# pyani-plus/pyani-plus

Hardware: AMD Instinct MI355X
Metric: pairwise genome comparisons/sec (N x N ANI matrix) (higher is better)
Workload: dtype u64

## Files before the change

pyani_plus_amd/csrc/capi.hip:

```cpp
#include <algorithm>
#include <cstdarg>
#include <cstring>

#include "pa_internal.h"

static thread_local char g_err[1024] = "";

void pa_set_error(const char *fmt, ...) {
  va_list ap;
  va_start(ap, fmt);
  vsnprintf(g_err, sizeof(g_err), fmt, ap);
  va_end(ap);
}

static hipEvent_t take_event(pa_ctx *c) {
  if (!c->event_pool.empty()) {
    hipEvent_t e = c->event_pool.back();
    c->event_pool.pop_back();
    return e;
  }
  hipEvent_t e = nullptr;
  if (hipEventCreate(&e) != hipSuccess) return nullptr;
  return e;
}

ProfScope::ProfScope(pa_ctx *ctx, int ph) : c(ctx), phase(ph) {
  if (!c->prof_on) return;
  e0 = take_event(c);
  e1 = take_event(c);
  if (e0) (void)hipEventRecord(e0, c->stream);
}

ProfScope::~ProfScope() {
  if (!c->prof_on || !e0 || !e1) return;
  (void)hipEventRecord(e1, c->stream);
  c->prof[phase].pending.emplace_back(e0, e1);
}

extern "C" {

int pa_abi_version(void) { return PA_ABI_VERSION; }
const char *pa_last_error(void) { return g_err; }

int pa_device_count(void) {
  int n = 0;
  if (hipGetDeviceCount(&n) != hipSuccess) return 0;
  return n;
}

int pa_ctx_create(int device, pa_ctx **out) {
  PA_REQUIRE(out != nullptr, "pa_ctx_create: out is null");
  *out = nullptr;
  int n = 0;
  hipError_t e = hipGetDeviceCount(&n);
  if (e != hipSuccess || n <= 0) {
    pa_set_error("no HIP device available (%s); libpyani_hip has no CPU fallback",
                 e != hipSuccess ? hipGetErrorString(e) : "device count is 0");
    return PA_E_NODEVICE;
  }
  PA_REQUIRE(device >= 0 && device < n, "pa_ctx_create: device %d out of range [0,%d)", device, n);
  PA_HIP(hipSetDevice(device));
  pa_ctx *c = new (std::nothrow) pa_ctx();
  if (!c) { pa_set_error("out of host memory"); return PA_E_NOMEM; }
  c->device = device;
  if (hipGetDeviceProperties(&c->prop, device) != hipSuccess) { delete c; pa_set_error("hipGetDeviceProperties failed"); return PA_E_HIP; }
  if (strncmp(c->prop.gcnArchName, "gfx950", 6) != 0) {
    pa_set_error("device %d is %s; this library is built for gfx950 (MI355X) only", device, c->prop.gcnArchName);
    delete c;
    return PA_E_NODEVICE;
  }
  if (hipStreamCreateWithFlags(&c->stream, hipStreamNonBlocking) != hipSuccess) { delete c; pa_set_error("hipStreamCreate failed"); return PA_E_HIP; }
  c->own_stream = true;
  if (hipHostMalloc(reinterpret_cast<void **>(&c->h_pinned), 64, hipHostMallocDefault) != hipSuccess) {
    (void)hipStreamDestroy(c->stream); delete c; pa_set_error("hipHostMalloc failed"); return PA_E_NOMEM;
  }
  if (c->counters.reserve(64) != PA_OK) { (void)hipHostFree(c->h_pinned); (void)hipStreamDestroy(c->stream); delete c; return PA_E_NOMEM; }
  *out = c;
  return PA_OK;
}

void pa_ctx_destroy(pa_ctx *c) {
  if (!c) return;
  (void)hipSetDevice(c->device);
  (void)hipStreamSynchronize(c->stream);
  DevBuf *bufs[] = {&c->cand_keys[0], &c->cand_keys[1], &c->cand_vals[0], &c->cand_vals[1], &c->genome_blk,
                    &c->counters, &c->hist, &c->flags, &c->scan_tmp, &c->region_off, &c->region_cursor, &c->dirty, &c->dict_keys[0], &c->dict_keys[1],
                    &c->dict_vals[0], &c->dict_vals[1], &c->ids, &c->post_genome, &c->bitrows, &c->dict_scalars, &c->cls_i, &c->cls_j, &c->cls_score,
                    &c->cls_cov};
  for (DevBuf *b : bufs) b->release();
  pa_fragani_release(c);
  for (auto &ph : c->prof)
    for (auto &pr : ph.pending) { (void)hipEventDestroy(pr.first); (void)hipEventDestroy(pr.second); }
  for (hipEvent_t e : c->event_pool) (void)hipEventDestroy(e);
  if (c->h_pinned) (void)hipHostFree(c->h_pinned);
  if (c->copy_stream) { (void)hipStreamSynchronize(c->copy_stream); (void)hipStreamDestroy(c->copy_stream); c->copy_stream = nullptr; }
  if (c->own_stream && c->stream) (void)hipStreamDestroy(c->stream);
  delete c;
}

int pa_ctx_set_stream(pa_ctx *c, void *hip_stream) {
  PA_REQUIRE(c != nullptr, "null context");
  PA_HIP(hipStreamSynchronize(c->stream));
  if (c->own_stream && c->stream) (void)hipStreamDestroy(c->stream);
  c->stream = reinterpret_cast<hipStream_t>(hip_stream);
  c->own_stream = false;
  return PA_OK;
}

int pa_ctx_own_stream(pa_ctx *c) {
  PA_REQUIRE(c != nullptr, "null context");
  if (c->own_stream) return PA_OK;
  PA_HIP(hipStreamSynchronize(c->stream));
  PA_HIP(hipStreamCreateWithFlags(&c->stream, hipStreamNonBlocking));
  c->own_stream = true;
  return PA_OK;
}

int pa_ctx_sync(pa_ctx *c) {
  PA_REQUIRE(c != nullptr, "null context");
  PA_HIP(hipStreamSynchronize(c->stream));
  return PA_OK;
}

int pa_ctx_device_info(pa_ctx *c, char *name256, int *compute_units, uint64_t *global_mem) {
  PA_REQUIRE(c != nullptr, "null context");
  if (name256) { snprintf(name256, 256, "%s (%s)", c->prop.name, c->prop.gcnArchName); }
  if (compute_units) *compute_units = c->prop.multiProcessorCount;
  if (global_mem) *global_mem = (uint64_t)c->prop.totalGlobalMem;
  return PA_OK;
}

int pa_dev_alloc(pa_ctx *c, uint64_t bytes, void **d_out) {
  PA_REQUIRE(c && d_out, "pa_dev_alloc: null argument");
  PA_HIP(hipSetDevice(c->device));
  hipError_t e = hipMalloc(d_out, bytes ? bytes : 16);
  if (e != hipSuccess) { pa_set_error("hipMalloc(%llu) failed: %s", (unsigned long long)bytes, hipGetErrorString(e)); return PA_E_NOMEM; }
  return PA_OK;
}
int pa_dev_free(pa_ctx *c, void *d_ptr) {
  PA_REQUIRE(c != nullptr, "null context");
  if (d_ptr) { PA_HIP(hipStreamSynchronize(c->stream)); PA_HIP(hipFree(d_ptr)); }
  return PA_OK;
}
int pa_memcpy_h2d(pa_ctx *c, void *d_dst, const void *h_src, uint64_t bytes) {
  PA_REQUIRE(c != nullptr, "null context");
  if (bytes == 0) return PA_OK;
  PA_HIP(hipMemcpyAsync(d_dst, h_src, bytes, hipMemcpyHostToDevice, c->stream));
  PA_HIP(hipStreamSynchronize(c->stream));
  return PA_OK;
}
int pa_memcpy_d2h(pa_ctx *c, void *h_dst, const void *d_src, uint64_t bytes) {
  PA_REQUIRE(c != nullptr, "null context");
  if (bytes == 0) return PA_OK;
  PA_HIP(hipMemcpyAsync(h_dst, d_src, bytes, hipMemcpyDeviceToHost, c->stream));
  PA_HIP(hipStreamSynchronize(c->stream));
  return PA_OK;
}
int pa_memset_d(pa_ctx *c, void *d_dst, int value, uint64_t bytes) {
  PA_REQUIRE(c != nullptr, "null context");
  if (bytes == 0) return PA_OK;
  PA_HIP(hipMemsetAsync(d_dst, value, bytes, c->stream));
  return PA_OK;
}

int pa_sketch(pa_ctx *c, const uint32_t *d_packed, const uint32_t *d_mask, const uint64_t *d_dirty_in, uint64_t arena_bases,
              const uint64_t *h_genome_start, uint32_t n_genomes, uint32_t k, uint64_t max_hash, uint64_t *d_hashes,
              uint64_t cap_hashes, uint64_t *d_off, uint64_t *h_total) {
  PA_REQUIRE(c && d_off && h_total && h_genome_start, "pa_sketch: null argument");
  PA_REQUIRE((arena_bases % PA_ALIGN_BASES) == 0, "pa_sketch: arena_bases %llu is not a multiple of %u",
             (unsigned long long)arena_bases, PA_ALIGN_BASES);
  PA_REQUIRE(arena_bases == 0 || (d_packed && d_mask), "pa_sketch: null arena");
  PA_REQUIRE(k >= 1 && k <= PA_MAX_K, "pa_sketch: k=%u outside [1,%u]", k, PA_MAX_K);
  PA_REQUIRE(h_genome_start[n_genomes] == arena_bases, "pa_sketch: genome_start[n] must equal arena_bases");
  PA_HIP(hipSetDevice(c->device));
  *h_total = 0;
  const uint64_t n_blocks = arena_bases / PA_ALIGN_BASES;
  std::vector<uint32_t> blk(n_genomes + 1);
  for (uint32_t g = 0; g <= n_genomes; ++g) {
    const uint64_t s = h_genome_start[g];
    PA_REQUIRE((s % PA_ALIGN_BASES) == 0 && (g == 0 || s >= h_genome_start[g - 1]) && s <= arena_bases,
               "pa_sketch: genome_start[%u]=%llu must be an ascending multiple of %u inside the arena", g,
               (unsigned long long)s, PA_ALIGN_BASES);
    blk[g] = (uint32_t)(s / PA_ALIGN_BASES);
  }
  PA_REQUIRE(n_blocks < (1ULL << 32), "pa_sketch: arena too large");
  PA_TRY(c->genome_blk.reserve((uint64_t)(n_genomes + 1) * sizeof(uint32_t)));
  PA_HIP(hipMemcpyAsync(c->genome_blk.p, blk.data(), (uint64_t)(n_genomes + 1) * sizeof(uint32_t),
                        hipMemcpyHostToDevice, c->stream));
  const double frac = (max_hash == UINT64_MAX) ? 1.0 : ((double)max_hash + 1.0) / 18446744073709551616.0;
  static const bool force_global = [] {
    const char *v = PA_TOOL_ENV("PA_SKETCH_SORT");
    return v && v[0] == 'g';
  }();
  std::vector<uint64_t> region_off(n_genomes + 1, 0);
  uint64_t longest_region = 0;
  for (uint32_t g = 0; g < n_genomes; ++g) {
    const uint64_t room = (uint64_t)((double)(h_genome_start[g + 1] - h_genome_start[g]) * frac * 1.25) + 128;
    longest_region = std::max(longest_region, room);
    region_off[g + 1] = region_off[g] + room;
  }
  const bool use_regions = !force_global && n_genomes > 0 && longest_region <= kLdsSortMax;
  if (use_regions) {
    PA_TRY(c->region_off.reserve((uint64_t)(n_genomes + 1) * sizeof(uint64_t)));
    PA_TRY(c->region_cursor.reserve((uint64_t)n_genomes * sizeof(uint32_t)));
    PA_HIP(hipMemcpyAsync(c->region_off.p, region_off.data(), (uint64_t)(n_genomes + 1) * sizeof(uint64_t),
                          hipMemcpyHostToDevice, c->stream));
  }
  const uint64_t *d_dirty = nullptr;
  PA_TRY(pa_dirty_or_build(c, d_mask, n_blocks, d_dirty_in, &d_dirty));
  PA_HIP(hipStreamSynchronize(c->stream));

  if (use_regions) {
    uint32_t *d_overflow = c->counters.as<uint32_t>() + 12;
    PA_TRY(c->cand_keys[0].reserve(region_off[n_genomes] * sizeof(uint64_t)));
    PA_HIP(hipMemsetAsync(c->region_cursor.p, 0, (uint64_t)n_genomes * sizeof(uint32_t), c->stream));
    PA_HIP(hipMemsetAsync(d_overflow, 0, sizeof(uint32_t), c->stream));
    {
      ProfScope prof(c, PA_PROF_KMER_HASH);
      PA_TRY(pa_launch_kmer_hash(c, d_packed, d_mask, d_dirty, n_blocks, c->genome_blk.as<uint32_t>(), n_genomes, k, max_hash,
                                 c->cand_keys[0].as<uint64_t>(), nullptr, 0, nullptr, c->region_off.as<uint64_t>(),
                                 c->region_cursor.as<uint32_t>(), d_overflow));
    }
    bool overflow = false;
    {
      ProfScope prof(c, PA_PROF_SKETCH_SORT);
      const int st = pa_sketch_from_regions(c, c->cand_keys[0].as<uint64_t>(), c->region_off.as<uint64_t>(),
                                            c->region_cursor.as<uint32_t>(), d_overflow, n_genomes,
                                            (uint32_t)longest_region, max_hash, d_hashes, cap_hashes, d_off, h_total, &overflow);
      if (st != PA_OK) return st;
    }
    if (!overflow) return PA_OK;
    *h_total = 0;
  }
  uint64_t cap = (uint64_t)((double)arena_bases * frac * 1.25) + 65536;
  if (cap > arena_bases) cap = arena_bases;
  uint64_t *d_count = c->counters.as<uint64_t>();
  uint64_t n_cand = 0;
  for (int attempt = 0; attempt < 2; ++attempt) {
    for (int b = 0; b < 2; ++b) {
      PA_TRY(c->cand_keys[b].reserve(cap * sizeof(uint64_t)));
      PA_TRY(c->cand_vals[b].reserve(cap * sizeof(uint32_t)));
    }
    PA_HIP(hipMemsetAsync(d_count, 0, sizeof(uint64_t), c->stream));
    {
      ProfScope prof(c, PA_PROF_KMER_HASH);
      PA_TRY(pa_launch_kmer_hash(c, d_packed, d_mask, d_dirty, n_blocks, c->genome_blk.as<uint32_t>(), n_genomes, k, max_hash,
                                 c->cand_keys[0].as<uint64_t>(), c->cand_vals[0].as<uint32_t>(), cap, d_count));
    }
    PA_HIP(hipMemcpyAsync(c->h_pinned, d_count, sizeof(uint64_t), hipMemcpyDeviceToHost, c->stream));
    PA_HIP(hipStreamSynchronize(c->stream));
    n_cand = c->h_pinned[0];
    if (n_cand <= cap) break;
    PA_REQUIRE(attempt == 0, "pa_sketch: candidate count changed between runs (%llu > %llu)",
               (unsigned long long)n_cand, (unsigned long long)cap);
    cap = n_cand;
  }
  {
    ProfScope prof(c, PA_PROF_SKETCH_SORT);
    uint64_t *keys[2] = {c->cand_keys[0].as<uint64_t>(), c->cand_keys[1].as<uint64_t>()};
    uint32_t *vals[2] = {c->cand_vals[0].as<uint32_t>(), c->cand_vals[1].as<uint32_t>()};
    int which = 0;
    int hash_bits = max_hash ? 64 - __builtin_clzll(max_hash) : 0;
    hash_bits = (hash_bits + 7) & ~7;
    int genome_bits = n_genomes > 1 ? 32 - __builtin_clz(n_genomes - 1) : 0;
    genome_bits = (genome_bits + 7) & ~7;
    PA_TRY(pa_radix_sort_pairs(c, keys, vals, n_cand, 0, hash_bits, false, &which));
    PA_TRY(pa_radix_sort_pairs(c, keys, vals, n_cand, 0, genome_bits, true, &which));
    int st = pa_build_sketch_csr(c, keys[which], vals[which], n_cand, n_genomes, d_hashes, cap_hashes, d_off, h_total);
    if (st != PA_OK) return st;
  }
  return PA_OK;
}

int pa_pair_counts_ex(pa_ctx *c, const uint64_t *d_hashes, const uint64_t *d_off, const uint64_t *h_off, uint32_t n,
                      uint32_t q0, uint32_t q1, uint32_t s0, uint32_t s1, uint32_t *d_counts, int algo) {
  PA_REQUIRE(c && d_off, "pa_pair_counts: null argument");
  PA_REQUIRE(q0 <= q1 && q1 <= n && s0 <= s1 && s1 <= n, "pa_pair_counts: ranges [%u,%u) x [%u,%u) outside [0,%u)", q0,
             q1, s0, s1, n);
  PA_REQUIRE(algo == PA_PAIRS_AUTO || algo == PA_PAIRS_BITROW || algo == PA_PAIRS_MERGE || algo == PA_PAIRS_BITROW_HASH,
             "pa_pair_counts: unknown algo %d", algo);
  PA_HIP(hipSetDevice(c->device));
  if (q0 == q1 || s0 == s1) { c->dict_prepared = false; return PA_OK; }
  PA_REQUIRE(d_counts != nullptr, "pa_pair_counts: null counts buffer");
  uint64_t total = 0;
  if (h_off) {
    total = h_off[n];
  } else {
    PA_HIP(hipMemcpyAsync(c->h_pinned, d_off + n, sizeof(uint64_t), hipMemcpyDeviceToHost, c->stream));
    PA_HIP(hipStreamSynchronize(c->stream));
    total = c->h_pinned[0];
  }
  PA_REQUIRE(total == 0 || d_hashes, "pa_pair_counts: null hashes");
  if (algo != PA_PAIRS_AUTO && algo != PA_PAIRS_BITROW_HASH) c->dict_prepared = false;
  switch (algo) {
    case PA_PAIRS_AUTO:
    case PA_PAIRS_BITROW_HASH:
      return pa_pairs_bitrow_hash(c, d_hashes, d_off, h_off, n, total, q0, q1, s0, s1, d_counts);
    case PA_PAIRS_BITROW:
      return pa_pairs_bitrow(c, d_hashes, d_off, n, total, q0, q1, s0, s1, d_counts);
    case PA_PAIRS_MERGE:
      return pa_pairs_merge(c, d_hashes, d_off, n, q0, q1, s0, s1, d_counts);
    default:
      pa_set_error("pa_pair_counts: unknown algo %d", algo);
      return PA_E_INVALID;
  }
}

int pa_pair_counts(pa_ctx *c, const uint64_t *d_hashes, const uint64_t *d_off, uint32_t n, uint32_t q0, uint32_t q1,
                   uint32_t s0, uint32_t s1, uint32_t *d_counts, int algo) {
  return pa_pair_counts_ex(c, d_hashes, d_off, nullptr, n, q0, q1, s0, s1, d_counts, algo);
}

int pa_pair_dict_prepare(pa_ctx *c, const uint64_t *d_subject_hashes, uint64_t n_postings) {
  PA_REQUIRE(c && (n_postings == 0 || d_subject_hashes), "pa_pair_dict_prepare: null argument");
  PA_HIP(hipSetDevice(c->device));
  return pa_pair_dict_prepare_impl(c, d_subject_hashes, n_postings);
}

int pa_ani(pa_ctx *c, const uint32_t *d_counts, const uint64_t *d_off, uint32_t q0, uint32_t q1, uint32_t s0,
           uint32_t s1, uint32_t k, double *d_identity, double *d_cov_query) {
  PA_REQUIRE(c && d_counts && d_off && d_identity && d_cov_query, "pa_ani: null argument");
  PA_REQUIRE(k >= 1 && q0 <= q1 && s0 <= s1, "pa_ani: bad k or ranges");
  PA_HIP(hipSetDevice(c->device));
  return pa_launch_ani(c, d_counts, d_off, q0, q1, s0, s1, k, d_identity, d_cov_query);
}

int pa_prof_enable(pa_ctx *c, int on) {
  PA_REQUIRE(c != nullptr, "null context");
  c->prof_on = on != 0;
  return PA_OK;
}

static int prof_drain(pa_ctx *c) {
  PA_HIP(hipStreamSynchronize(c->stream));
  for (auto &ph : c->prof) {
    for (auto &pr : ph.pending) {
      float ms = 0.f;
      if (hipEventElapsedTime(&ms, pr.first, pr.second) == hipSuccess) {
        ph.total_ms += ms;
        ph.launches += 1;
      }
      c->event_pool.push_back(pr.first);
      c->event_pool.push_back(pr.second);
    }
    ph.pending.clear();
  }
  return PA_OK;
}

int pa_prof_reset(pa_ctx *c) {
  PA_REQUIRE(c != nullptr, "null context");
  PA_TRY(prof_drain(c));
  for (auto &ph : c->prof) { ph.total_ms = 0.0; ph.launches = 0; }
  return PA_OK;
}

int pa_prof_get(pa_ctx *c, int phase, double *total_ms, uint64_t *launches) {
  PA_REQUIRE(c != nullptr && phase >= 0 && phase < PA_PROF_NPHASES, "pa_prof_get: bad phase %d", phase);
  PA_TRY(prof_drain(c));
  if (total_ms) *total_ms = c->prof[phase].total_ms;
  if (launches) *launches = c->prof[phase].launches;
  return PA_OK;
}

}
```

pyani_plus_amd/csrc/kmer_hash.hip:

```cpp
#include <cstdlib>
#include <type_traits>

#include "pa_internal.h"
#include "murmur_dev.h"

namespace {

using namespace pa_dev;

constexpr int kThreads = 256;
constexpr uint32_t kStageCap = 1024;

constexpr int pow2_floor(int k) { int c = 1; while (2 * c <= k) c *= 2; return c; }

__device__ __forceinline__ uint32_t find_genome(const uint32_t *__restrict__ genome_blk, uint32_t n, uint32_t blk) {
  uint32_t lo = 0, hi = n;
  while (hi - lo > 1) {
    uint32_t mid = (lo + hi) >> 1;
    if (genome_blk[mid] <= blk) lo = mid; else hi = mid;
  }
  return lo;
}

__device__ __forceinline__ void region_append(uint64_t *__restrict__ regions, const uint64_t *__restrict__ region_off,
                                              uint32_t *__restrict__ cursor, uint32_t *__restrict__ overflow,
                                              uint32_t g, uint64_t h) {
  const uint64_t slot = atomicAdd(&cursor[g], 1u);
  if (slot < region_off[g + 1] - region_off[g]) regions[region_off[g] + slot] = h; else *overflow = 1u;
}

template <int K, bool LUT>
__global__ __launch_bounds__(kThreads) void kmer_hash_kernel(
    const uint4 *__restrict__ packed, const uint2 *__restrict__ mask, const uint64_t *__restrict__ dirty, uint32_t n_blocks64,
    const uint32_t *__restrict__ genome_blk, uint32_t n_genomes, uint64_t max_hash,
    uint64_t *__restrict__ cand_hash, uint32_t *__restrict__ cand_genome, uint64_t cap,
    unsigned long long *__restrict__ count, const uint64_t *__restrict__ region_off, uint32_t *__restrict__ cursor,
    uint32_t *__restrict__ overflow, uint32_t blk0) {
  static_assert(K >= 1 && K <= 32, "a k-mer is one 64-bit register pair");
  __shared__ uint64_t s_hash[kStageCap];
  __shared__ uint32_t s_blk[kStageCap];
  __shared__ uint32_t s_n;
  __shared__ unsigned long long s_base;
  constexpr int kWords = (K + 7) / 8;
  __shared__ uint64_t s_lo[LUT ? kWords : 1][256];
  __shared__ uint32_t s_hi[LUT ? kWords : 1][256];

  const uint32_t tid = threadIdx.x;
  const uint32_t max_hi = (uint32_t)(max_hash >> 32);
  const bool take_all = max_hi == 0xffffffffu;
  const uint32_t screen_hi = max_hi + 1u;
  if (tid == 0) s_n = 0;
  if constexpr (LUT) {
#pragma unroll
    for (int j = 0; j < kWords; ++j) {
      const uint64_t cj = (j & 1) ? kC2 : kC1;
      s_lo[j][tid] = (uint64_t)ascii_group(tid, K - 8 * j) * cj;
      s_hi[j][tid] = (uint32_t)((uint64_t)ascii_group(tid, K - 8 * j - 4) * cj);
    }
  }
  __syncthreads();

  const uint32_t t = blk0 + blockIdx.x * kThreads + tid;
  if (t < n_blocks64) {
    const uint4 cur = packed[t];
    uint2 pw = make_uint2(0u, 0u);
    if (t > 0) pw = reinterpret_cast<const uint2 *>(packed)[2 * (uint64_t)t - 1];
    uint32_t d1 = 0u, d2 = 0u;
    const uint32_t wave_blk = __builtin_amdgcn_readfirstlane(t & ~63u);
    const uint64_t dirty_word = dirty[wave_blk >> 6];
    if ((dirty_word >> (t & 63u)) & 1ull) {
      const uint2 m = mask[t];
      uint32_t d0 = t > 0 ? mask[t - 1].y : 0xffffffffu;
      d1 = m.x;
      d2 = m.y;
      int c = 1;
#pragma unroll
      for (; 2 * c <= K; c *= 2) {
        d2 |= alignbit(d2, d1, 32 - c);
        d1 |= alignbit(d1, d0, 32 - c);
        d0 |= d0 << c;
      }
      constexpr int cc = pow2_floor(K);
      constexpr int r = K - cc;
      if constexpr (r > 0) {
        d2 |= alignbit(d2, d1, 32 - r);
        d1 |= alignbit(d1, d0, 32 - r);
      }
    }
    const uint32_t bad[2] = {d1, d2};
    if ((d1 & d2) != 0xffffffffu) {
      constexpr uint64_t kMask = (K == 32) ? ~0ULL : ((1ULL << (2 * K)) - 1);
      constexpr uint32_t kMaskHi = (uint32_t)(kMask >> 32);
      uint32_t fw[8] = {pw.x, pw.y, cur.x, cur.y, cur.z, cur.w, 0u, 0u};
      uint32_t rw[6];
#pragma unroll
      for (int j = 0; j < 6; ++j) {
        const uint32_t x = __builtin_bitreverse32(fw[5 - j]);
        rw[j] = ~(((x >> 1) & 0x55555555u) | ((x & 0x55555555u) << 1));
      }
      auto columns = [&](auto base_tag, int i_begin, int i_end) {
        constexpr int kBase = decltype(base_tag)::value;
#pragma unroll 1
        for (int i = i_begin; i < i_end; ++i) {
          constexpr int kOff = 33 - K;
          const uint32_t fo = 2u * (uint32_t)((i + kOff) & 15), ro = 30u - 2u * (uint32_t)i;
          uint32_t A[5], B[5];
#pragma unroll
          for (int j = 0; j < 5; ++j) {
            A[j] = alignbit(fw[kBase + j + 1], fw[kBase + j], fo);
            B[j] = alignbit(rw[j + 1], rw[j], ro);
          }
#pragma unroll
          for (int wi = 0; wi < 4; ++wi) {
            const uint32_t f_lo = A[wi], f_hi = A[wi + 1], r_lo = B[3 - wi], r_hi = B[4 - wi];
          const uint64_t f_lsb = u64_of(f_lo, f_hi) & kMask, r_lsb = u64_of(r_lo, r_hi) & kMask;
          const uint64_t fwd = __builtin_amdgcn_uicmpl(f_lsb, r_lsb, 37 );
          uint32_t clo, chi;
          asm("s_nop 1\n\tv_cndmask_b32_e64 %0, %1, %2, %3" : "=v"(clo) : "v"((uint32_t)r_lsb), "v"((uint32_t)f_lsb), "s"(fwd));
          asm("v_cndmask_b32_e64 %0, %1, %2, %3" : "=v"(chi) : "v"((uint32_t)(r_lsb >> 32)), "v"((uint32_t)(f_lsb >> 32)), "s"(fwd), "v"(clo));
          uint64_t P[4] = {0, 0, 0, 0};
#pragma unroll
          for (int j = 0; j < kWords; ++j) {
            const uint32_t src = j < 2 ? clo : chi;
            const uint32_t glo = (src >> (16 * (j & 1))) & 0xffu, ghi = (src >> (16 * (j & 1) + 8)) & 0xffu;
            if constexpr (LUT) {
              const uint64_t lo = s_lo[j][glo];
              const uint32_t hi = (uint32_t)(lo >> 32) + s_hi[j][ghi];
              P[j] = u64_of((uint32_t)lo, hi);
            } else {
              const uint64_t word = u64_of(ascii_group(glo, K - 8 * j), ascii_group(ghi, K - 8 * j - 4));
              P[j] = word * ((j & 1) ? kC2 : kC1);
            }
          }
          (void)kMaskHi;
          uint64_t U, V;
          murmur3_pre_last_mul<K>(P, U, V);
          if (take_all || last_mul_high_sum_plus1(U, V) <= screen_hi) {
            const uint64_t X = U * kF2, Y = V * kF2;
            const uint64_t h = (X ^ (X >> 33)) + (Y ^ (Y >> 33));
            if (h > max_hash || ((bad[wi >> 1] >> (16 * (wi & 1) + i)) & 1u)) continue;
            const uint32_t slot = atomicAdd(&s_n, 1u);
            if (slot < kStageCap) {
              s_hash[slot] = h;
              s_blk[slot] = t;
            } else if (region_off) {
              region_append(cand_hash, region_off, cursor, overflow, find_genome(genome_blk, n_genomes, t), h);
            } else {
              const unsigned long long g = atomicAdd(count, 1ULL);
              if (g < cap) {
                cand_hash[g] = h;
                cand_genome[g] = find_genome(genome_blk, n_genomes, t);
              }
            }
          }
          }
        }
      };
      constexpr int kOff0 = 33 - K, kSplit = (kOff0 & 15) ? 16 - (kOff0 & 15) : 16;
      columns(std::integral_constant<int, (kOff0 >> 4)>{}, 0, kSplit);
      if constexpr (kSplit < 16) columns(std::integral_constant<int, (kOff0 >> 4) + 1>{}, kSplit, 16);
    }
  }
  __syncthreads();
  const uint32_t n = min(s_n, kStageCap);
  if (n == 0) return;
  if (region_off) {
    const uint32_t b0 = blk0 + blockIdx.x * kThreads;
    const uint32_t b1 = min(b0 + (uint32_t)kThreads, n_blocks64) - 1u;
    const uint32_t g0 = find_genome(genome_blk, n_genomes, b0);
    if (genome_blk[g0 + 1] > b1) {
      if (tid == 0) s_base = atomicAdd(&cursor[g0], n);
      __syncthreads();
      const uint64_t room = region_off[g0 + 1] - region_off[g0];
      uint64_t *__restrict__ dst = cand_hash + region_off[g0];
      for (uint32_t i = tid; i < n; i += kThreads) {
        const uint64_t slot = s_base + i;
        if (slot < room) dst[slot] = s_hash[i]; else *overflow = 1u;
      }
    } else {
      for (uint32_t i = tid; i < n; i += kThreads)
        region_append(cand_hash, region_off, cursor, overflow, find_genome(genome_blk, n_genomes, s_blk[i]), s_hash[i]);
    }
    return;
  }
  if (tid == 0) s_base = atomicAdd(count, (unsigned long long)n);
  __syncthreads();
  const unsigned long long base = s_base;
  for (uint32_t i = tid; i < n; i += kThreads) {
    const unsigned long long g = base + i;
    if (g < cap) {
      cand_hash[g] = s_hash[i];
      cand_genome[g] = find_genome(genome_blk, n_genomes, s_blk[i]);
    }
  }
}

template <int K, bool LUT>
int launch_variant(pa_ctx *c, const uint32_t *d_packed, const uint32_t *d_mask, const uint64_t *d_dirty, uint64_t n_blocks64,
           const uint32_t *d_genome_blk, uint32_t n_genomes, uint64_t max_hash, uint64_t *d_cand_hash,
           uint32_t *d_cand_genome, uint64_t cap, uint64_t *d_count, const uint64_t *d_region_off, uint32_t *d_cursor,
           uint32_t *d_overflow, uint64_t blk0, hipStream_t stream) {
  const uint32_t grid = ceil_div_u64(n_blocks64 - blk0, kThreads);
  hipLaunchKernelGGL((kmer_hash_kernel<K, LUT>), dim3(grid), dim3(kThreads), 0, stream ? stream : c->stream,
                     reinterpret_cast<const uint4 *>(d_packed), reinterpret_cast<const uint2 *>(d_mask), d_dirty,
                     (uint32_t)n_blocks64, d_genome_blk, n_genomes, max_hash, d_cand_hash, d_cand_genome, cap,
                     reinterpret_cast<unsigned long long *>(d_count), d_region_off, d_cursor, d_overflow, (uint32_t)blk0);
  PA_HIP(hipGetLastError());
  return PA_OK;
}

template <int K>
int launch(pa_ctx *c, const uint32_t *d_packed, const uint32_t *d_mask, const uint64_t *d_dirty, uint64_t n_blocks64,
           const uint32_t *d_genome_blk, uint32_t n_genomes, uint64_t max_hash, uint64_t *d_cand_hash,
           uint32_t *d_cand_genome, uint64_t cap, uint64_t *d_count, const uint64_t *d_region_off, uint32_t *d_cursor,
           uint32_t *d_overflow, uint64_t blk0, hipStream_t stream) {
  static const bool arithmetic = [] {
    const char *v = PA_TOOL_ENV("PA_KMER_VARIANT");
    return v && v[0] == '0';
  }();
  if constexpr (K == 31)
    if (arithmetic)
      return launch_variant<K, false>(c, d_packed, d_mask, d_dirty, n_blocks64, d_genome_blk, n_genomes, max_hash, d_cand_hash,
                                    d_cand_genome, cap, d_count, d_region_off, d_cursor, d_overflow, blk0, stream);
  return launch_variant<K, true>(c, d_packed, d_mask, d_dirty, n_blocks64, d_genome_blk, n_genomes, max_hash, d_cand_hash,
                                 d_cand_genome, cap, d_count, d_region_off, d_cursor, d_overflow, blk0, stream);
}

template <int K>
__global__ __launch_bounds__(kThreads) void kmer_hash_wide_kernel(
    const uint4 *__restrict__ packed, const uint2 *__restrict__ mask, const uint64_t *__restrict__ dirty, uint32_t n_blocks64,
    const uint32_t *__restrict__ genome_blk, uint32_t n_genomes, uint64_t max_hash,
    uint64_t *__restrict__ cand_hash, uint32_t *__restrict__ cand_genome, uint64_t cap,
    unsigned long long *__restrict__ count, const uint64_t *__restrict__ region_off, uint32_t *__restrict__ cursor,
    uint32_t *__restrict__ overflow, uint32_t blk0) {
  static_assert(K >= 33 && K <= 64, "k-mers of 65 to 128 bits");
  __shared__ uint64_t s_hash[kStageCap];
  __shared__ uint32_t s_blk[kStageCap];
  __shared__ uint32_t s_n;
  __shared__ unsigned long long s_base;
  constexpr int kWords = (K + 7) / 8;
  __shared__ uint64_t s_lo[kWords][256];
  __shared__ uint32_t s_hi[kWords][256];
  const uint32_t tid = threadIdx.x;
  const uint32_t max_hi = (uint32_t)(max_hash >> 32);
  const bool take_all = max_hi == 0xffffffffu;
  const uint32_t screen_hi = max_hi + 1u;
  if (tid == 0) s_n = 0;
#pragma unroll
  for (int j = 0; j < kWords; ++j) {
    const uint64_t cj = (j & 1) ? kC2 : kC1;
    s_lo[j][tid] = (uint64_t)ascii_group(tid, K - 8 * j) * cj;
    s_hi[j][tid] = (uint32_t)((uint64_t)ascii_group(tid, K - 8 * j - 4) * cj);
  }
  __syncthreads();

  const uint32_t t = blk0 + blockIdx.x * kThreads + tid;
  if (t < n_blocks64) {
    const uint4 cur = packed[t];
    const uint4 prev = t > 0 ? packed[t - 1] : make_uint4(0u, 0u, 0u, 0u);
    uint32_t d2 = 0u, d3 = 0u;
    const uint32_t wave_blk = __builtin_amdgcn_readfirstlane(t & ~63u);
    const uint64_t dirty_word = dirty[wave_blk >> 6];
    const uint64_t before = wave_blk ? dirty[(wave_blk >> 6) - 1] >> 63 : 1ull;
    const uint64_t dirty_or_prev = dirty_word | (dirty_word << 1) | before;
    if ((dirty_or_prev >> (t & 63u)) & 1ull) {
      const uint2 m = mask[t];
      uint32_t d0 = 0xffffffffu, d1 = 0xffffffffu;
      if (t > 0) { const uint2 mp = mask[t - 1]; d0 = mp.x; d1 = mp.y; }
      d2 = m.x;
      d3 = m.y;
#pragma unroll
      for (int c = 1; c <= 16; c *= 2) {
        d3 |= alignbit(d3, d2, 32 - c);
        d2 |= alignbit(d2, d1, 32 - c);
        d1 |= alignbit(d1, d0, 32 - c);
        d0 |= d0 << c;
      }
      if constexpr (K == 64) {
        d3 |= d2; d2 |= d1; d1 |= d0;
      } else {
        constexpr int r = K - 32;
        d3 |= alignbit(d3, d2, 32 - r);
        d2 |= alignbit(d2, d1, 32 - r);
        d1 |= alignbit(d1, d0, 32 - r);
      }
    }
    const uint32_t bad[2] = {d2, d3};
    if ((d2 & d3) != 0xffffffffu) {
      constexpr uint32_t kMask2 = (2 * K - 64 >= 32) ? 0xffffffffu : ((1u << (2 * K - 64)) - 1u);
      constexpr uint32_t kMask3 = (2 * K - 96 >= 32) ? 0xffffffffu : (2 * K - 96 <= 0 ? 0u : ((1u << ((2 * K - 96) & 31)) - 1u));
      const uint32_t fw[10] = {prev.x, prev.y, prev.z, prev.w, cur.x, cur.y, cur.z, cur.w, 0u, 0u};
      uint32_t rw[10];
#pragma unroll
      for (int j = 0; j < 10; ++j) {
        const uint32_t x = __builtin_bitreverse32(fw[9 - j]);
        rw[j] = ~(((x >> 1) & 0x55555555u) | ((x & 0x55555555u) << 1));
      }
      auto columns = [&](auto base_tag, int i_begin, int i_end) {
        constexpr int kBase = decltype(base_tag)::value;
#pragma unroll 1
        for (int i = i_begin; i < i_end; ++i) {
          constexpr int kOff = 65 - K;
          const uint32_t fo = 2u * (uint32_t)((i + kOff) & 15), ro = 30u - 2u * (uint32_t)i;
          uint32_t A[7], B[7];
#pragma unroll
          for (int j = 0; j < 7; ++j) {
            A[j] = alignbit(fw[kBase + j + 1], fw[kBase + j], fo);
            B[j] = alignbit(rw[j + 3], rw[j + 2], ro);
          }
#pragma unroll
          for (int wi = 0; wi < 4; ++wi) {
            const uint32_t f0 = A[wi], f1 = A[wi + 1], f2 = A[wi + 2] & kMask2, f3 = A[wi + 3] & kMask3;
            const uint32_t r0 = B[3 - wi], r1 = B[4 - wi], r2 = B[5 - wi] & kMask2, r3 = B[6 - wi] & kMask3;
            const uint64_t lt_hi = __builtin_amdgcn_uicmpl(u64_of(f2, f3), u64_of(r2, r3), 36 );
            const uint64_t eq_hi = __builtin_amdgcn_uicmpl(u64_of(f2, f3), u64_of(r2, r3), 32 );
            const uint64_t le_lo = __builtin_amdgcn_uicmpl(u64_of(f0, f1), u64_of(r0, r1), 37 );
            const uint64_t fwd = lt_hi | (eq_hi & le_lo);
            uint32_t c0, c1, c2, c3;
            asm("s_nop 1\n\tv_cndmask_b32_e64 %0, %1, %2, %3" : "=v"(c0) : "v"(r0), "v"(f0), "s"(fwd));
            asm("v_cndmask_b32_e64 %0, %1, %2, %3" : "=v"(c1) : "v"(r1), "v"(f1), "s"(fwd), "v"(c0));
            asm("v_cndmask_b32_e64 %0, %1, %2, %3" : "=v"(c2) : "v"(r2), "v"(f2), "s"(fwd), "v"(c1));
            asm("v_cndmask_b32_e64 %0, %1, %2, %3" : "=v"(c3) : "v"(r3), "v"(f3), "s"(fwd), "v"(c2));
            const uint32_t cw[4] = {c0, c1, c2, c3};
            uint64_t P[8] = {0, 0, 0, 0, 0, 0, 0, 0};
#pragma unroll
            for (int j = 0; j < kWords; ++j) {
              const uint32_t src = cw[j >> 1];
              const uint32_t glo = (src >> (16 * (j & 1))) & 0xffu, ghi = (src >> (16 * (j & 1) + 8)) & 0xffu;
              const uint64_t lo = s_lo[j][glo];
              P[j] = u64_of((uint32_t)lo, (uint32_t)(lo >> 32) + s_hi[j][ghi]);
            }
            uint64_t U, V;
            murmur3_pre_last_mul<K>(P, U, V);
            if (take_all || last_mul_high_sum_plus1(U, V) <= screen_hi) {
              const uint64_t X = U * kF2, Y = V * kF2;
              const uint64_t h = (X ^ (X >> 33)) + (Y ^ (Y >> 33));
              if (h > max_hash || ((bad[wi >> 1] >> (16 * (wi & 1) + i)) & 1u)) continue;
              const uint32_t slot = atomicAdd(&s_n, 1u);
              if (slot < kStageCap) {
                s_hash[slot] = h;
                s_blk[slot] = t;
              } else if (region_off) {
                region_append(cand_hash, region_off, cursor, overflow, find_genome(genome_blk, n_genomes, t), h);
              } else {
                const unsigned long long g = atomicAdd(count, 1ULL);
                if (g < cap) {
                  cand_hash[g] = h;
                  cand_genome[g] = find_genome(genome_blk, n_genomes, t);
                }
              }
            }
          }
        }
      };
      constexpr int kOff0 = 65 - K, kSplit = (kOff0 & 15) ? 16 - (kOff0 & 15) : 16;
      columns(std::integral_constant<int, (kOff0 >> 4)>{}, 0, kSplit);
      if constexpr (kSplit < 16) columns(std::integral_constant<int, (kOff0 >> 4) + 1>{}, kSplit, 16);
    }
  }
  __syncthreads();
  const uint32_t n = min(s_n, kStageCap);
  if (n == 0) return;
  if (region_off) {
    const uint32_t b0 = blk0 + blockIdx.x * kThreads;
    const uint32_t b1 = min(b0 + (uint32_t)kThreads, n_blocks64) - 1u;
    const uint32_t g0 = find_genome(genome_blk, n_genomes, b0);
    if (genome_blk[g0 + 1] > b1) {
      if (tid == 0) s_base = atomicAdd(&cursor[g0], n);
      __syncthreads();
      const uint64_t room = region_off[g0 + 1] - region_off[g0];
      uint64_t *__restrict__ dst = cand_hash + region_off[g0];
      for (uint32_t i = tid; i < n; i += kThreads) {
        const uint64_t slot = s_base + i;
        if (slot < room) dst[slot] = s_hash[i]; else *overflow = 1u;
      }
    } else {
      for (uint32_t i = tid; i < n; i += kThreads)
        region_append(cand_hash, region_off, cursor, overflow, find_genome(genome_blk, n_genomes, s_blk[i]), s_hash[i]);
    }
    return;
  }
  if (tid == 0) s_base = atomicAdd(count, (unsigned long long)n);
  __syncthreads();
  const unsigned long long base = s_base;
  for (uint32_t i = tid; i < n; i += kThreads) {
    const unsigned long long g = base + i;
    if (g < cap) {
      cand_hash[g] = s_hash[i];
      cand_genome[g] = find_genome(genome_blk, n_genomes, s_blk[i]);
    }
  }
}

__device__ __forceinline__ uint32_t rev_groups32(uint32_t x) {
  x = __builtin_bitreverse32(x);
  return ((x >> 1) & 0x55555555u) | ((x & 0x55555555u) << 1);
}

__device__ __forceinline__ void murmur3_pre_last_mul_rt(const uint64_t (&P)[8], uint32_t k, uint64_t &U, uint64_t &V) {
  uint64_t h1 = 42, h2 = 42;
  const uint32_t nblocks = k >> 4, tail = k & 15u;
#pragma unroll
  for (uint32_t i = 0; i < 4; ++i) {
    if (i >= nblocks) break;
    h1 ^= rotl64(P[2 * i], 31) * kC2;
    h1 = rotl64(h1, 27) + h2;
    h1 = times5_plus(h1, 0x52dce729ULL);
    h2 ^= rotl64(P[2 * i + 1], 33) * kC1;
    h2 = rotl64(h2, 31) + h1;
    h2 = times5_plus(h2, 0x38495ab5ULL);
  }
  uint64_t t1 = 0, t2 = 0;
#pragma unroll
  for (uint32_t i = 0; i < 4; ++i)
    if (i == nblocks) { t1 = P[2 * i]; t2 = P[2 * i + 1]; }
  if (tail > 8) h2 ^= rotl64(t2, 33) * kC1;
  if (tail > 0) h1 ^= rotl64(t1, 31) * kC2;
  h1 ^= (uint64_t)k;
  h2 ^= (uint64_t)k;
  h1 += h2;
  h2 += h1;
  h1 ^= h1 >> 33; h1 *= kF1; h1 ^= h1 >> 33;
  h2 ^= h2 >> 33; h2 *= kF1; h2 ^= h2 >> 33;
  U = h1;
  V = h2;
}

constexpr int kLongIter = 32;
__global__ __launch_bounds__(kThreads) void kmer_hash_long_kernel(
    const uint32_t *__restrict__ packed, const uint32_t *__restrict__ mask, uint64_t pos0, uint64_t pos1, uint32_t k,
    const uint32_t *__restrict__ genome_blk, uint32_t n_genomes, uint64_t max_hash, uint64_t *__restrict__ cand_hash,
    uint32_t *__restrict__ cand_genome, uint64_t cap, unsigned long long *__restrict__ count,
    const uint64_t *__restrict__ region_off, uint32_t *__restrict__ cursor, uint32_t *__restrict__ overflow) {
  __shared__ uint64_t s_lo[8][256];
  __shared__ uint32_t s_hi[8][256];
  const uint32_t tid = threadIdx.x;
  const uint32_t n_words = (k + 7u) >> 3;
  for (uint32_t j = 0; j < n_words; ++j) {
    const uint64_t cj = (j & 1u) ? kC2 : kC1;
    s_lo[j][tid] = (uint64_t)ascii_group(tid, (int)k - 8 * (int)j) * cj;
    s_hi[j][tid] = (uint32_t)((uint64_t)ascii_group(tid, (int)k - 8 * (int)j - 4) * cj);
  }
  __syncthreads();
  const uint64_t wg_first = pos0 + ((uint64_t)blockIdx.y * gridDim.x + blockIdx.x) * (uint64_t)(kThreads * kLongIter);
#pragma unroll 1
  for (int it = 0; it < kLongIter; ++it) {
  const uint64_t e = wg_first + (uint64_t)it * kThreads + tid;
  if (e >= pos1 || e + 1 < k) continue;
  const uint64_t a = e + 1 - k;
  {
    const uint64_t m0 = a >> 5, m_last = e >> 5;
    const uint32_t sm = (uint32_t)(a & 31u);
    const uint32_t w0 = mask[m0], w1 = m0 + 1 <= m_last ? mask[m0 + 1] : 0u, w2 = m0 + 2 <= m_last ? mask[m0 + 2] : 0u;
    const uint32_t b0 = alignbit(w1, w0, sm), b1 = alignbit(w2, w1, sm);
    const uint32_t top = k == 64 ? 0xffffffffu : ((1u << (k - 32u)) - 1u);
    if (b0 | (b1 & top)) continue;
  }
  uint32_t F[4], R[4];
  {
    const uint64_t p0 = a >> 4, p_last = e >> 4;
    const uint32_t sp = 2u * (uint32_t)(a & 15u);
    uint32_t w[5];
#pragma unroll
    for (int i = 0; i < 5; ++i) w[i] = p0 + i <= p_last ? packed[p0 + i] : 0u;
#pragma unroll
    for (int i = 0; i < 4; ++i) F[i] = alignbit(w[i + 1], w[i], sp);
    const uint32_t used = 2u * k - 64u;
    if (used < 32u) { F[2] &= (1u << used) - 1u; F[3] = 0u; }
    else if (used < 64u) F[3] &= (1u << (used - 32u)) - 1u;
    const uint32_t C[6] = {~rev_groups32(F[3]), ~rev_groups32(F[2]), ~rev_groups32(F[1]), ~rev_groups32(F[0]), 0u, 0u};
    const uint32_t s = 128u - 2u * k, ws = s >> 5, bs = s & 31u;
#pragma unroll
    for (int i = 0; i < 4; ++i) R[i] = ws ? alignbit(C[i + 2], C[i + 1], bs) : alignbit(C[i + 1], C[i], bs);
    if (used < 32u) { R[2] &= (1u << used) - 1u; R[3] = 0u; }
    else if (used < 64u) R[3] &= (1u << (used - 32u)) - 1u;
  }
  const uint64_t f_hi = u64_of(F[2], F[3]), f_lo = u64_of(F[0], F[1]), r_hi = u64_of(R[2], R[3]), r_lo = u64_of(R[0], R[1]);
  const bool fwd = f_hi < r_hi || (f_hi == r_hi && f_lo <= r_lo);
  uint32_t c[4];
#pragma unroll
  for (int i = 0; i < 4; ++i) c[i] = fwd ? F[i] : R[i];
  uint64_t P[8] = {0, 0, 0, 0, 0, 0, 0, 0};
#pragma unroll
  for (uint32_t j = 0; j < 8; ++j) {
    if (j >= n_words) break;
    const uint32_t src = c[j >> 1], glo = (src >> (16u * (j & 1u))) & 0xffu, ghi = (src >> (16u * (j & 1u) + 8u)) & 0xffu;
    const uint64_t lo = s_lo[j][glo];
    P[j] = u64_of((uint32_t)lo, (uint32_t)(lo >> 32) + s_hi[j][ghi]);
  }
  uint64_t U, V;
  murmur3_pre_last_mul_rt(P, k, U, V);
  const uint32_t max_hi = (uint32_t)(max_hash >> 32);
  if (max_hi != 0xffffffffu && last_mul_high_sum_plus1(U, V) > max_hi + 1u) continue;
  const uint64_t X = U * kF2, Y = V * kF2;
  const uint64_t h = (X ^ (X >> 33)) + (Y ^ (Y >> 33));
  if (h > max_hash) continue;
  const uint32_t blk = (uint32_t)(e >> 6);
  const uint32_t g = find_genome(genome_blk, n_genomes, blk);
  if (region_off) {
    region_append(cand_hash, region_off, cursor, overflow, g, h);
  } else {
    const unsigned long long slot = atomicAdd(count, 1ULL);
    if (slot < cap) {
      cand_hash[slot] = h;
      cand_genome[slot] = g;
    }
  }
  }
}

}

int pa_launch_kmer_hash(pa_ctx *c, const uint32_t *d_packed, const uint32_t *d_mask, const uint64_t *d_dirty, uint64_t n_blocks64,
                        const uint32_t *d_genome_blk, uint32_t n_genomes, uint32_t k, uint64_t max_hash,
                        uint64_t *d_cand_hash, uint32_t *d_cand_genome, uint64_t cap, uint64_t *d_count,
                        const uint64_t *d_region_off, uint32_t *d_cursor, uint32_t *d_overflow, uint64_t blk0,
                        hipStream_t stream) {
  PA_REQUIRE(n_blocks64 < (1ULL << 32), "arena too large: %llu blocks of 64 bases", (unsigned long long)n_blocks64);
  if (n_blocks64 <= blk0) return PA_OK;
  const char *long_form = PA_TOOL_ENV("PA_KMER_LONG");
  const bool long_plain = long_form && long_form[0] == 'p';
  if (k > 32 && k <= 64 && !long_plain) {
    PA_REQUIRE((blk0 & 63u) == 0, "k-mer hash launch must start at a multiple of 64 blocks, not %llu", (unsigned long long)blk0);
    const uint32_t grid = ceil_div_u64(n_blocks64 - blk0, kThreads);
#define PA_WIDE_CASE(KK)                                                                                                   \
  case KK:                                                                                                                 \
    hipLaunchKernelGGL((kmer_hash_wide_kernel<KK>), dim3(grid), dim3(kThreads), 0, stream ? stream : c->stream,            \
                       reinterpret_cast<const uint4 *>(d_packed), reinterpret_cast<const uint2 *>(d_mask), d_dirty,        \
                       (uint32_t)n_blocks64, d_genome_blk, n_genomes, max_hash, d_cand_hash, d_cand_genome, cap,           \
                       reinterpret_cast<unsigned long long *>(d_count), d_region_off, d_cursor, d_overflow, (uint32_t)blk0); \
    break;
    switch (k) {
      PA_WIDE_CASE(33) PA_WIDE_CASE(34) PA_WIDE_CASE(35) PA_WIDE_CASE(36) PA_WIDE_CASE(37) PA_WIDE_CASE(38) PA_WIDE_CASE(39)
      PA_WIDE_CASE(40) PA_WIDE_CASE(41) PA_WIDE_CASE(42) PA_WIDE_CASE(43) PA_WIDE_CASE(44) PA_WIDE_CASE(45) PA_WIDE_CASE(46)
      PA_WIDE_CASE(47) PA_WIDE_CASE(48) PA_WIDE_CASE(49) PA_WIDE_CASE(50) PA_WIDE_CASE(51) PA_WIDE_CASE(52) PA_WIDE_CASE(53)
      PA_WIDE_CASE(54) PA_WIDE_CASE(55) PA_WIDE_CASE(56) PA_WIDE_CASE(57) PA_WIDE_CASE(58) PA_WIDE_CASE(59) PA_WIDE_CASE(60)
      PA_WIDE_CASE(61) PA_WIDE_CASE(62) PA_WIDE_CASE(63) PA_WIDE_CASE(64)
      default: break;
    }
#undef PA_WIDE_CASE
    PA_HIP(hipGetLastError());
    return PA_OK;
  }
  if (k > 32 && k <= 64) {
    const uint64_t pos0 = blk0 * 64, pos1 = n_blocks64 * 64;
    const uint64_t per_wg = (uint64_t)kThreads * kLongIter;
    const uint64_t n_wg = (pos1 - pos0 + per_wg - 1) / per_wg;
    const uint32_t gx = (uint32_t)std::min<uint64_t>(n_wg, 1u << 20), gy = (uint32_t)((n_wg + gx - 1) / gx);
    PA_REQUIRE(gy <= 65535u, "arena too large for one launch of the long k-mer kernel: %llu positions", (unsigned long long)(pos1 - pos0));
    hipLaunchKernelGGL(kmer_hash_long_kernel, dim3(gx, gy), dim3(kThreads), 0,
                       stream ? stream : c->stream, d_packed, d_mask, pos0, pos1, k, d_genome_blk, n_genomes, max_hash,
                       d_cand_hash, d_cand_genome, cap, reinterpret_cast<unsigned long long *>(d_count), d_region_off,
                       d_cursor, d_overflow);
    PA_HIP(hipGetLastError());
    return PA_OK;
  }
#define PA_K_CASE(KK) \
  case KK: return launch<KK>(c, d_packed, d_mask, d_dirty, n_blocks64, d_genome_blk, n_genomes, max_hash, d_cand_hash, d_cand_genome, cap, d_count, d_region_off, d_cursor, d_overflow, blk0, stream);
  PA_REQUIRE((blk0 & 63u) == 0, "k-mer hash launch must start at a multiple of 64 blocks, not %llu", (unsigned long long)blk0);
  switch (k) {
    PA_K_CASE(1) PA_K_CASE(2) PA_K_CASE(3) PA_K_CASE(4) PA_K_CASE(5) PA_K_CASE(6) PA_K_CASE(7) PA_K_CASE(8)
    PA_K_CASE(9) PA_K_CASE(10) PA_K_CASE(11) PA_K_CASE(12) PA_K_CASE(13) PA_K_CASE(14) PA_K_CASE(15) PA_K_CASE(16)
    PA_K_CASE(17) PA_K_CASE(18) PA_K_CASE(19) PA_K_CASE(20) PA_K_CASE(21) PA_K_CASE(22) PA_K_CASE(23) PA_K_CASE(24)
    PA_K_CASE(25) PA_K_CASE(26) PA_K_CASE(27) PA_K_CASE(28) PA_K_CASE(29) PA_K_CASE(30) PA_K_CASE(31) PA_K_CASE(32)
    default:
      pa_set_error("k=%u outside [1,64]", k);
      return PA_E_INVALID;
  }
#undef PA_K_CASE
}
```

pyani_plus_amd/csrc/murmur_dev.h:

```cpp
#pragma once

#include <hip/hip_runtime.h>

#include <cstdint>

namespace pa_dev {

__device__ __forceinline__ uint32_t alignbit(uint32_t hi, uint32_t lo, uint32_t sh) {
  return __builtin_amdgcn_alignbit(hi, lo, sh);
}

__device__ __forceinline__ uint32_t ascii4(uint32_t b8) {
  uint32_t u = (b8 | (b8 << 12)) & 0x000F000Fu;
  uint32_t v = (u | (u << 6)) & 0x03030303u;
  return __builtin_amdgcn_perm(0u, 0x54474341u, v);
}

__device__ __forceinline__ uint64_t u64_of(uint32_t lo, uint32_t hi) { return ((uint64_t)hi << 32) | lo; }

__device__ __forceinline__ uint64_t rotl64(uint64_t x, int r) {
  const uint32_t lo = (uint32_t)x, hi = (uint32_t)(x >> 32);
  if (r == 32) return u64_of(hi, lo);
  if (r < 32) return u64_of(alignbit(lo, hi, 32 - r), alignbit(hi, lo, 32 - r));
  return u64_of(alignbit(hi, lo, 64 - r), alignbit(lo, hi, 64 - r));
}

__device__ __forceinline__ uint64_t fmix64(uint64_t k) {
  k ^= k >> 33;
  k *= 0xff51afd7ed558ccdULL;
  k ^= k >> 33;
  k *= 0xc4ceb9fe1a85ec53ULL;
  k ^= k >> 33;
  return k;
}

constexpr uint64_t kC1 = 0x87c37b91114253d5ULL, kC2 = 0x4cf5ad432745937fULL;

__device__ __forceinline__ uint64_t times5_plus(uint64_t h, uint64_t c) {
  uint64_t t;
  asm("v_lshl_add_u64 %0, %1, 2, %1" : "=v"(t) : "v"(h));
  return t + c;
}

constexpr uint64_t kF1 = 0xff51afd7ed558ccdULL, kF2 = 0xc4ceb9fe1a85ec53ULL;

template <int K, int N>
__device__ __forceinline__ void murmur3_pre_last_mul(const uint64_t (&P)[N], uint64_t &U, uint64_t &V) {
  static_assert(N >= (K + 7) / 8, "one first product per 8-byte word of the k-mer");
  uint64_t h1 = 42, h2 = 42;
  constexpr int nblocks = K / 16;
  constexpr int tail = K % 16;
#pragma unroll
  for (int i = 0; i < nblocks; ++i) {
    const uint64_t k1 = rotl64(P[2 * i], 31) * kC2;
    h1 ^= k1;
    if (i == 0) {
      h1 = times5_plus(rotl64(h1, 27), 5ULL * 42ULL + 0x52dce729ULL);
    } else {
      h1 = rotl64(h1, 27) + h2;
      h1 = times5_plus(h1, 0x52dce729ULL);
    }
    const uint64_t k2 = rotl64(P[2 * i + 1], 33) * kC1;
    h2 ^= k2;
    h2 = rotl64(h2, 31) + h1;
    h2 = times5_plus(h2, 0x38495ab5ULL);
  }
  if constexpr (tail > 8) h2 ^= rotl64(P[2 * nblocks + 1], 33) * kC1;
  if constexpr (tail > 0) h1 ^= rotl64(P[2 * nblocks], 31) * kC2;
  h1 ^= (uint64_t)K; h2 ^= (uint64_t)K;
  h1 += h2; h2 += h1;
  h1 ^= h1 >> 33; h1 *= kF1; h1 ^= h1 >> 33;
  h2 ^= h2 >> 33; h2 *= kF1; h2 ^= h2 >> 33;
  U = h1;
  V = h2;
}

__device__ __forceinline__ uint32_t last_mul_high_sum_plus1(uint64_t U, uint64_t V) {
  constexpr uint32_t c0 = (uint32_t)kF2, c1 = (uint32_t)(kF2 >> 32);
  const uint32_t u0 = (uint32_t)U, u1 = (uint32_t)(U >> 32), v0 = (uint32_t)V, v1 = (uint32_t)(V >> 32);
  return (__umulhi(u0, c0) + __umulhi(v0, c0) + 1u) + ((u0 + v0) * c1 + (u1 + v1) * c0);
}

template <int K, int N>
__device__ __forceinline__ uint64_t murmur3_from_products(const uint64_t (&P)[N]) {
  uint64_t U, V;
  murmur3_pre_last_mul<K, N>(P, U, V);
  const uint64_t X = U * kF2, Y = V * kF2;
  return (X ^ (X >> 33)) + (Y ^ (Y >> 33));
}

__device__ __forceinline__ uint32_t ascii_group(uint32_t b8, int nv) {
  const uint32_t a = ascii4(b8);
  return nv >= 4 ? a : (nv <= 0 ? 0u : (a & ((1u << (8 * nv)) - 1u)));
}

}
```

pyani_plus_amd/csrc/pa_internal.h:

```cpp
#pragma once

#include <hip/hip_runtime.h>

#include <cstdarg>
#include <cstdint>
#include <cstdio>
#include <string>
#include <vector>

#include "../../include/pyani_hip.h"

void pa_set_error(const char *fmt, ...);

#define PA_HIP(call)                                                                          \
  do {                                                                                        \
    hipError_t _e = (call);                                                                   \
    if (_e != hipSuccess) {                                                                   \
      pa_set_error("%s failed: %s (%s:%d)", #call, hipGetErrorString(_e), __FILE__, __LINE__); \
      return PA_E_HIP;                                                                        \
    }                                                                                         \
  } while (0)

#define PA_TRY(call)          \
  do {                        \
    int _s = (call);          \
    if (_s != PA_OK) return _s; \
  } while (0)

#define PA_REQUIRE(cond, ...)   \
  do {                          \
    if (!(cond)) {              \
      pa_set_error(__VA_ARGS__); \
      return PA_E_INVALID;      \
    }                           \
  } while (0)

#ifdef PA_TOOLS
#include <cstdlib>
#define PA_TOOL_ENV(name) getenv(name)
#else
#define PA_TOOL_ENV(name) static_cast<const char *>(nullptr)
#endif

struct DevBudget {
  uint64_t held = 0, peak = 0, cap = 0;
  char what[192] = {0};
};
struct DevBuf {
  void *p = nullptr;
  uint64_t bytes = 0;
  DevBudget *budget = nullptr;
  int reserve(uint64_t want) {
    if (want <= bytes) return PA_OK;
    uint64_t sz = want + want / 4 + 256;
    if (budget && budget->cap && budget->held - bytes + sz > budget->cap) {
      pa_set_error("%s: the workspace would grow to %llu bytes (%llu held; this buffer from %llu to %llu), above the cap of %llu bytes",
                   budget->what[0] ? budget->what : "device workspace", (unsigned long long)(budget->held - bytes + sz),
                   (unsigned long long)budget->held, (unsigned long long)bytes, (unsigned long long)sz, (unsigned long long)budget->cap);
      return PA_E_NOMEM;
    }
    if (p) (void)hipFree(p);
    if (budget) budget->held -= bytes;
    p = nullptr;
    bytes = 0;
    hipError_t e = hipMalloc(&p, sz);
    if (e != hipSuccess) {
      if (budget)
        pa_set_error("%s: hipMalloc(%llu) failed with %llu bytes of workspace held: %s", budget->what[0] ? budget->what : "device workspace",
                     (unsigned long long)sz, (unsigned long long)budget->held, hipGetErrorString(e));
      else
        pa_set_error("hipMalloc(%llu) failed: %s", (unsigned long long)sz, hipGetErrorString(e));
      p = nullptr;
      return PA_E_NOMEM;
    }
    bytes = sz;
    if (budget) {
      budget->held += sz;
      if (budget->held > budget->peak) budget->peak = budget->held;
    }
    return PA_OK;
  }
  void release() {
    if (p) (void)hipFree(p);
    if (budget) budget->held -= bytes;
    p = nullptr;
    bytes = 0;
  }
  template <typename T>
  T *as() const { return reinterpret_cast<T *>(p); }
};

struct ProfPhase {
  double total_ms = 0.0;
  uint64_t launches = 0;
  std::vector<std::pair<hipEvent_t, hipEvent_t>> pending;
};

struct pa_ctx {
  int device = 0;
  hipStream_t stream = nullptr;
  bool own_stream = false;
  hipDeviceProp_t prop;
  DevBuf cand_keys[2], cand_vals[2];
  DevBuf genome_blk;
  DevBuf counters;
  DevBuf hist;
  DevBuf flags, scan_tmp;
  DevBuf region_off, region_cursor;
  DevBuf dirty;
  DevBuf dict_keys[2], dict_vals[2];
  DevBuf ids, post_genome, bitrows;
  bool dict_prepared = false;
  uint64_t dict_prepared_postings = 0;
  uint32_t dict_prepared_cap = 0;
  DevBuf dict_scalars;
  hipStream_t copy_stream = nullptr;
  DevBuf cls_i, cls_j, cls_score, cls_cov;
  void *frag_work = nullptr;
  uint64_t *h_pinned = nullptr;
  bool prof_on = false;
  ProfPhase prof[PA_PROF_NPHASES];
  std::vector<hipEvent_t> event_pool;
};

struct ProfScope {
  pa_ctx *c;
  int phase;
  hipEvent_t e0 = nullptr, e1 = nullptr;
  ProfScope(pa_ctx *ctx, int ph);
  ~ProfScope();
};

static inline uint32_t ceil_div_u64(uint64_t a, uint64_t b) { return (uint32_t)((a + b - 1) / b); }

int pa_radix_sort_pairs(pa_ctx *c, uint64_t *keys[2], uint32_t *vals[2], uint64_t n, int bit_lo,
                        int bit_hi, bool by_val, int *which);
int pa_exclusive_scan_u32(pa_ctx *c, const uint32_t *d_in, uint32_t *d_out, uint64_t n,
                          uint64_t *d_total_u64 );

void pa_fragani_release(pa_ctx *c);

int pa_launch_kmer_hash(pa_ctx *c, const uint32_t *d_packed, const uint32_t *d_mask, const uint64_t *d_dirty, uint64_t n_blocks64,
                        const uint32_t *d_genome_blk, uint32_t n_genomes, uint32_t k, uint64_t max_hash,
                        uint64_t *d_cand_hash, uint32_t *d_cand_genome, uint64_t cap, uint64_t *d_count,
                        const uint64_t *d_region_off = nullptr, uint32_t *d_cursor = nullptr,
                        uint32_t *d_overflow = nullptr, uint64_t blk0 = 0, hipStream_t stream = nullptr);

int pa_build_dirty(pa_ctx *c, const uint32_t *d_mask, uint64_t n_blocks64, uint64_t *d_dirty, hipStream_t stream = nullptr);
int pa_dirty_or_build(pa_ctx *c, const uint32_t *d_mask, uint64_t n_blocks64, const uint64_t *d_dirty, const uint64_t **out);

constexpr uint32_t kLdsSortMax = 16384;
int pa_sketch_from_regions(pa_ctx *c, uint64_t *d_regions, const uint64_t *d_region_off, const uint32_t *d_cursor,
                           const uint32_t *d_overflow, uint32_t n_genomes, uint32_t longest_region, uint64_t max_hash,
                           uint64_t *d_hashes, uint64_t cap_hashes, uint64_t *d_off, uint64_t *h_total, bool *h_overflow);

int pa_build_sketch_csr(pa_ctx *c, const uint64_t *d_sorted_hash, const uint32_t *d_sorted_genome,
                        uint64_t n_cand, uint32_t n_genomes, uint64_t *d_hashes, uint64_t cap_hashes,
                        uint64_t *d_off, uint64_t *h_total);

int pa_pairs_bitrow(pa_ctx *c, const uint64_t *d_hashes, const uint64_t *d_off, uint32_t n, uint64_t total,
                    uint32_t q0, uint32_t q1, uint32_t s0, uint32_t s1, uint32_t *d_counts);
int pa_dense_ids_sorted(pa_ctx *c, const uint64_t *d_hashes, const uint64_t *d_off, uint32_t n, uint64_t P,
                        uint64_t *n_distinct);
int pa_pairs_bitrow_hash(pa_ctx *c, const uint64_t *d_hashes, const uint64_t *d_off, const uint64_t *h_off ,
                         uint32_t n, uint64_t total, uint32_t q0, uint32_t q1, uint32_t s0, uint32_t s1,
                         uint32_t *d_counts);
int pa_pair_dict_prepare_impl(pa_ctx *c, const uint64_t *d_subject_hashes, uint64_t n_postings);
int pa_pairs_merge(pa_ctx *c, const uint64_t *d_hashes, const uint64_t *d_off, uint32_t n, uint32_t q0,
                   uint32_t q1, uint32_t s0, uint32_t s1, uint32_t *d_counts);

int pa_launch_ani(pa_ctx *c, const uint32_t *d_counts, const uint64_t *d_off, uint32_t q0, uint32_t q1,
                  uint32_t s0, uint32_t s1, uint32_t k, double *d_identity, double *d_cov_query);
```

pyani_plus_amd/csrc/pairs_bitrow.hip:

```cpp
#include <algorithm>
#include <cstdlib>
#include <vector>

#include "pa_internal.h"

namespace {

constexpr int kThreads = 256;
constexpr int kPlanes = 10;
constexpr uint32_t kMaxTileSubjects = 2048;
constexpr uint32_t kNone = 0xffffffffu;
constexpr uint64_t kEmptyKey = ~0ULL;

__global__ __launch_bounds__(kThreads) void iota_kernel(uint32_t *__restrict__ vals, uint64_t n) {
  const uint64_t i = (uint64_t)blockIdx.x * kThreads + threadIdx.x;
  if (i < n) vals[i] = (uint32_t)i;
}

__global__ __launch_bounds__(kThreads) void last_or_kernel(const uint64_t *__restrict__ hashes,
                                                           const uint64_t *__restrict__ off, uint32_t n,
                                                           unsigned long long *__restrict__ or_out) {
  const uint32_t g = blockIdx.x * kThreads + threadIdx.x;
  uint64_t k = 0;
  if (g < n && off[g + 1] > off[g]) k = hashes[off[g + 1] - 1];
#pragma unroll
  for (int o = 32; o > 0; o >>= 1) k |= __shfl_xor(k, o, 64);
  if ((threadIdx.x & 63u) == 0 && k) atomicOr(or_out, (unsigned long long)k);
}

__global__ __launch_bounds__(kThreads) void key_heads_kernel(const uint64_t *__restrict__ keys, uint64_t n,
                                                             uint32_t *__restrict__ flags) {
  const uint64_t i = (uint64_t)blockIdx.x * kThreads + threadIdx.x;
  if (i < n) flags[i] = (i == 0 || keys[i] != keys[i - 1]) ? 1u : 0u;
}

__device__ __forceinline__ uint32_t owner_of(const uint64_t *__restrict__ off, uint32_t n, uint64_t j) {
  uint32_t lo = 0, hi = n;
  while (hi - lo > 1) {
    const uint32_t mid = (lo + hi) >> 1;
    if (off[mid] <= j) lo = mid; else hi = mid;
  }
  return lo;
}

__global__ __launch_bounds__(kThreads) void assign_ids_kernel(
    const uint32_t *__restrict__ sorted_post, const uint32_t *__restrict__ flags, const uint32_t *__restrict__ pos,
    uint64_t n, const uint64_t *__restrict__ off, uint32_t n_genomes, uint32_t *__restrict__ ids_csr,
    uint32_t *__restrict__ id_sorted, uint32_t *__restrict__ genome_sorted) {
  const uint64_t i = (uint64_t)blockIdx.x * kThreads + threadIdx.x;
  if (i >= n) return;
  const uint32_t id = pos[i] + flags[i] - 1u;
  const uint32_t j = sorted_post[i];
  ids_csr[j] = id;
  id_sorted[i] = id;
  genome_sorted[i] = owner_of(off, n_genomes, j);
}

__global__ __launch_bounds__(kThreads) void build_rows_kernel(const uint32_t *__restrict__ id_sorted,
                                                              const uint32_t *__restrict__ genome_sorted, uint64_t n,
                                                              uint32_t t0, uint32_t t1, uint32_t w32,
                                                              uint32_t *__restrict__ rows) {
  const uint64_t i = (uint64_t)blockIdx.x * kThreads + threadIdx.x;
  if (i >= n) return;
  const uint32_t g = genome_sorted[i];
  if (g < t0 || g >= t1) return;
  const uint32_t col = g - t0;
  atomicOr(&rows[(uint64_t)id_sorted[i] * w32 + (col >> 5)], 1u << (col & 31u));
}

struct U4 { uint32_t v[4]; };

template <int TPR>
__global__ __launch_bounds__(kThreads) void row_sum_kernel(const uint32_t *__restrict__ ids_csr,
                                                           const uint64_t *__restrict__ off, uint32_t q0,
                                                           const uint32_t *__restrict__ rows, uint32_t tile_cols,
                                                           uint32_t *__restrict__ counts, uint32_t ns,
                                                           uint32_t col0) {
  constexpr int kRowsPerIter = kThreads / TPR;
  constexpr int kW32 = TPR * 4;
  __shared__ uint32_t s_cnt[kW32 * 32];
  const uint32_t tid = threadIdx.x;
  for (uint32_t x = tid; x < kW32 * 32; x += kThreads) s_cnt[x] = 0;
  __syncthreads();

  const uint32_t q = q0 + blockIdx.x;
  const uint64_t beg = off[q], len = off[q + 1] - beg;
  const uint32_t *__restrict__ ids = ids_csr + beg;
  const uint32_t slot = tid / TPR, quad = tid % TPR;

  uint32_t plane[kPlanes][4];
#pragma unroll
  for (int p = 0; p < kPlanes; ++p)
#pragma unroll
    for (int c = 0; c < 4; ++c) plane[p][c] = 0;
  uint32_t pending = 0;

  auto flush = [&]() {
#pragma unroll
    for (int c = 0; c < 4; ++c) {
      uint32_t any = 0;
#pragma unroll
      for (int p = 0; p < kPlanes; ++p) any |= plane[p][c];
      while (any) {
        const uint32_t b = (uint32_t)__builtin_ctz(any);
        any &= any - 1u;
        uint32_t v = 0;
#pragma unroll
        for (int p = 0; p < kPlanes; ++p) v |= ((plane[p][c] >> b) & 1u) << p;
        atomicAdd(&s_cnt[(quad * 4 + c) * 32 + b], v);
      }
    }
#pragma unroll
    for (int p = 0; p < kPlanes; ++p)
#pragma unroll
      for (int c = 0; c < 4; ++c) plane[p][c] = 0;
    pending = 0;
  };

  constexpr int kBatch = 8;
  auto csa = [](uint32_t &carry, uint32_t &sum, uint32_t a, uint32_t b, uint32_t c) {
    const uint32_t u = a ^ b;
    carry = (a & b) | (u & c);
    sum = u ^ c;
  };
  const uint64_t j_begin = slot < (uint32_t)kRowsPerIter ? slot : len;
  uint32_t id_next[kBatch];
#pragma unroll
  for (int u = 0; u < kBatch; ++u) {
    const uint64_t j = j_begin + (uint64_t)u * kRowsPerIter;
    id_next[u] = j < len ? ids[j] : kNone;
  }
  for (uint64_t j0 = j_begin; j0 < len; j0 += (uint64_t)kRowsPerIter * kBatch) {
    uint4 r[kBatch];
#pragma unroll
    for (int u = 0; u < kBatch; ++u) {
      const uint32_t id = id_next[u];
      r[u] = id != kNone ? *reinterpret_cast<const uint4 *>(rows + (uint64_t)id * kW32 + quad * 4) : make_uint4(0u, 0u, 0u, 0u);
    }
#pragma unroll
    for (int u = 0; u < kBatch; ++u) {
      const uint64_t j = j0 + (uint64_t)(kBatch + u) * kRowsPerIter;
      id_next[u] = j < len ? ids[j] : kNone;
    }
#pragma unroll
    for (int c = 0; c < 4; ++c) {
      auto word = [&](int u) -> uint32_t { return c == 0 ? r[u].x : c == 1 ? r[u].y : c == 2 ? r[u].z : r[u].w; };
      uint32_t twos_a, twos_b, fours_a, fours_b, eights;
      csa(twos_a, plane[0][c], plane[0][c], word(0), word(1));
      csa(twos_b, plane[0][c], plane[0][c], word(2), word(3));
      csa(fours_a, plane[1][c], plane[1][c], twos_a, twos_b);
      csa(twos_a, plane[0][c], plane[0][c], word(4), word(5));
      csa(twos_b, plane[0][c], plane[0][c], word(6), word(7));
      csa(fours_b, plane[1][c], plane[1][c], twos_a, twos_b);
      csa(eights, plane[2][c], plane[2][c], fours_a, fours_b);
#pragma unroll
      for (int p = 3; p < kPlanes; ++p) {
        const uint32_t t = plane[p][c] & eights;
        plane[p][c] ^= eights;
        eights = t;
      }
    }
    pending += kBatch;
    if (pending + kBatch > (1u << kPlanes) - 1u) flush();
  }
  if (pending) flush();
  __syncthreads();
  uint32_t *__restrict__ out = counts + (uint64_t)blockIdx.x * ns + col0;
  for (uint32_t x = tid; x < tile_cols; x += kThreads) out[x] = s_cnt[x];
}

__global__ __launch_bounds__(kThreads) void zero_rows_kernel(uint4 *__restrict__ rows, const uint32_t *__restrict__ d_u,
                                                             uint32_t w32) {
  const uint64_t n16 = ((uint64_t)(*d_u ? *d_u : 1u) * w32) / 4u;
  const uint64_t i = (uint64_t)blockIdx.x * kThreads + threadIdx.x;
  if (i < n16) rows[i] = make_uint4(0u, 0u, 0u, 0u);
}

struct DictEntry {
  unsigned long long key;
  uint32_t id;
  uint32_t pad;
};
static_assert(sizeof(DictEntry) == 16, "one probe = one 16-byte entry");

__device__ __forceinline__ uint32_t slot_of(uint64_t h, uint32_t cap) {
  const uint32_t x = ((uint32_t)h * 0x9E3779B1u) ^ (uint32_t)(h >> 32);
  return (uint32_t)(((uint64_t)x * cap) >> 32);
}

constexpr int kInsertPerThread = 4;
__global__ __launch_bounds__(kThreads) void table_insert_kernel(const uint64_t *__restrict__ hashes, uint64_t p0,
                                                                uint64_t p1, DictEntry *__restrict__ table,
                                                                uint32_t cap, uint32_t *__restrict__ counter,
                                                                uint32_t *__restrict__ special) {
  __shared__ uint32_t s_won, s_base;
  if (threadIdx.x == 0) s_won = 0;
  __syncthreads();
  uint32_t won_slot[kInsertPerThread];
  int won = 0;
  bool won_special = false;
  const uint64_t base = p0 + (uint64_t)blockIdx.x * (kThreads * kInsertPerThread) + threadIdx.x;
#pragma unroll
  for (int i = 0; i < kInsertPerThread; ++i) {
    const uint64_t p = base + (uint64_t)i * kThreads;
    if (p >= p1) break;
    const uint64_t h = hashes[p];
    if (h == kEmptyKey) {
      won_special = atomicCAS(&special[0], kNone, kNone - 1u) == kNone;
      continue;
    }
    uint32_t slot = slot_of(h, cap);
    for (;;) {
      unsigned long long k = *reinterpret_cast<volatile const unsigned long long *>(&table[slot].key);
      if (k == kEmptyKey) k = atomicCAS(&table[slot].key, (unsigned long long)kEmptyKey, (unsigned long long)h);
      if (k == kEmptyKey) { won_slot[won++] = slot; break; }
      if (k == h) break;
      if (++slot == cap) slot = 0;
    }
  }
  const uint32_t mine = (uint32_t)won + (won_special ? 1u : 0u);
  uint32_t local = mine ? atomicAdd(&s_won, mine) : 0u;
  __syncthreads();
  if (threadIdx.x == 0) s_base = s_won ? atomicAdd(counter, s_won) : 0u;
  __syncthreads();
  local += s_base;
  for (int i = 0; i < won; ++i) table[won_slot[i]].id = local++;
  if (won_special) special[0] = local;
}

template <bool SET_BITS>
__global__ __launch_bounds__(kThreads) void table_lookup_kernel(
    const uint64_t *__restrict__ hashes, uint64_t p0, uint64_t p1, const DictEntry *__restrict__ table, uint32_t cap,
    const uint32_t *__restrict__ special, uint32_t *__restrict__ ids_csr, const uint64_t *__restrict__ off, uint32_t n,
    uint32_t t0, uint32_t w32, uint32_t *__restrict__ rows) {
  uint64_t p;
  if constexpr (SET_BITS) {
    const uint64_t beg = off[t0 + blockIdx.y];
    p = beg + (uint64_t)blockIdx.x * kThreads + threadIdx.x;
    if (p >= off[t0 + blockIdx.y + 1]) return;
  } else {
    p = p0 + (uint64_t)blockIdx.x * kThreads + threadIdx.x;
    if (p >= p1) return;
  }
  const uint64_t h = hashes[p];
  uint32_t id = kNone;
  if (h == kEmptyKey) {
    id = special[0];
  } else {
    uint32_t slot = slot_of(h, cap);
    for (;;) {
      const uint4 e = *reinterpret_cast<const uint4 *>(&table[slot]);
      const uint64_t k = ((uint64_t)e.y << 32) | e.x;
      if (k == h) { id = e.z; break; }
      if (k == kEmptyKey) break;
      if (++slot == cap) slot = 0;
    }
  }
  ids_csr[p] = id;
  if constexpr (SET_BITS) {
    const uint32_t col = blockIdx.y;
    atomicOr(&rows[(uint64_t)id * w32 + (col >> 5)], 1u << (col & 31u));
  }
}

__global__ __launch_bounds__(kThreads) void postings_fingerprint_kernel(const uint64_t *__restrict__ hashes, uint64_t n,
                                                                        unsigned long long *__restrict__ out) {
  uint64_t a = 0, b = 0;
  for (uint64_t i = (uint64_t)blockIdx.x * kThreads + threadIdx.x; i < n; i += (uint64_t)gridDim.x * kThreads) {
    const uint64_t h = hashes[i];
    a += h;
    b += (h ^ (h >> 29)) * 0x9E3779B97F4A7C15ULL;
  }
#pragma unroll
  for (int o = 32; o > 0; o >>= 1) { a += __shfl_xor(a, o, 64); b += __shfl_xor(b, o, 64); }
  if ((threadIdx.x & 63u) == 0) {
    atomicAdd(&out[0], (unsigned long long)a);
    atomicAdd(&out[1], (unsigned long long)b);
  }
}

__global__ __launch_bounds__(256) void mirror_lower_kernel(uint32_t *__restrict__ counts, uint32_t n, uint32_t tile) {
  __shared__ uint32_t s_t[32][33];
  const uint32_t r0 = blockIdx.y * 32u, c0 = blockIdx.x * 32u;
  if (r0 / tile <= c0 / tile) return;
  const uint32_t tx = threadIdx.x & 31u, ty = threadIdx.x >> 5;
  for (uint32_t y = ty; y < 32u; y += 8u) {
    const uint32_t sr = c0 + y, sc = r0 + tx;
    s_t[y][tx] = (sr < n && sc < n) ? counts[(uint64_t)sr * n + sc] : 0u;
  }
  __syncthreads();
  for (uint32_t y = ty; y < 32u; y += 8u) {
    const uint32_t dr = r0 + y, dc = c0 + tx;
    if (dr < n && dc < n) counts[(uint64_t)dr * n + dc] = s_t[tx][y];
  }
}

template <int TPR>
void launch_row_sum(pa_ctx *c, uint32_t nq, const uint32_t *ids, const uint64_t *off, uint32_t q0,
                    const uint32_t *rows, uint32_t tile_cols, uint32_t *counts, uint32_t ns, uint32_t col0) {
  hipLaunchKernelGGL(row_sum_kernel<TPR>, dim3(nq), dim3(kThreads), 0, c->stream, ids, off, q0, rows, tile_cols,
                     counts, ns, col0);
}

int dispatch_row_sum(pa_ctx *c, int tpr, uint32_t nq, const uint32_t *ids, const uint64_t *off, uint32_t q0,
                     const uint32_t *rows, uint32_t tile_cols, uint32_t *counts, uint32_t ns, uint32_t col0) {
#define PA_ROW_CASE(T) \
  case T: launch_row_sum<T>(c, nq, ids, off, q0, rows, tile_cols, counts, ns, col0); return PA_OK;
  switch (tpr) {
    PA_ROW_CASE(1) PA_ROW_CASE(2) PA_ROW_CASE(3) PA_ROW_CASE(4) PA_ROW_CASE(5) PA_ROW_CASE(6) PA_ROW_CASE(7)
    PA_ROW_CASE(8) PA_ROW_CASE(9) PA_ROW_CASE(10) PA_ROW_CASE(11) PA_ROW_CASE(12) PA_ROW_CASE(13) PA_ROW_CASE(14)
    PA_ROW_CASE(15) PA_ROW_CASE(16)
    default:
      pa_set_error("pair phase: %d threads per bit row (tile wider than %u subjects)", tpr, kMaxTileSubjects);
      return PA_E_INVALID;
  }
#undef PA_ROW_CASE
}

}

int pa_dense_ids_sorted(pa_ctx *c, const uint64_t *d_hashes, const uint64_t *d_off, uint32_t n, uint64_t P,
                        uint64_t *n_distinct) {
  ProfScope prof(c, PA_PROF_PAIR_DICT);
  for (int b = 0; b < 2; ++b) {
    PA_TRY(c->dict_keys[b].reserve(P * sizeof(uint64_t)));
    PA_TRY(c->dict_vals[b].reserve(P * sizeof(uint32_t)));
  }
  PA_TRY(c->ids.reserve(P * sizeof(uint32_t)));
  PA_TRY(c->post_genome.reserve(2 * P * sizeof(uint32_t)));
  PA_TRY(c->flags.reserve(2 * P * sizeof(uint32_t)));
  uint64_t *keys[2] = {c->dict_keys[0].as<uint64_t>(), c->dict_keys[1].as<uint64_t>()};
  uint32_t *vals[2] = {c->dict_vals[0].as<uint32_t>(), c->dict_vals[1].as<uint32_t>()};
  uint32_t *d_ids = c->ids.as<uint32_t>();
  uint32_t *d_id_sorted = c->post_genome.as<uint32_t>();
  uint32_t *d_genome_sorted = d_id_sorted + P;
  uint32_t *d_flags = c->flags.as<uint32_t>(), *d_pos = d_flags + P;
  uint64_t *d_scalars = c->counters.as<uint64_t>();

  const uint32_t grid = ceil_div_u64(P, kThreads);
  PA_HIP(hipMemcpyAsync(keys[0], d_hashes, P * sizeof(uint64_t), hipMemcpyDeviceToDevice, c->stream));
  PA_HIP(hipMemsetAsync(d_scalars + 2, 0, 2 * sizeof(uint64_t), c->stream));
  hipLaunchKernelGGL(iota_kernel, dim3(grid), dim3(kThreads), 0, c->stream, vals[0], P);
  hipLaunchKernelGGL(last_or_kernel, dim3(ceil_div_u64(n, kThreads)), dim3(kThreads), 0, c->stream, d_hashes, d_off,
                     n, reinterpret_cast<unsigned long long *>(d_scalars + 2));
  PA_HIP(hipMemcpyAsync(c->h_pinned, d_scalars + 2, sizeof(uint64_t), hipMemcpyDeviceToHost, c->stream));
  PA_HIP(hipStreamSynchronize(c->stream));
  const uint64_t all_or = c->h_pinned[0];
  int bit_hi = all_or ? 64 - __builtin_clzll(all_or) : 0;
  bit_hi = (bit_hi + 7) & ~7;
  int which = 0;
  PA_TRY(pa_radix_sort_pairs(c, keys, vals, P, 0, bit_hi, false, &which));
  hipLaunchKernelGGL(key_heads_kernel, dim3(grid), dim3(kThreads), 0, c->stream, keys[which], P, d_flags);
  PA_TRY(pa_exclusive_scan_u32(c, d_flags, d_pos, P, d_scalars + 3));
  hipLaunchKernelGGL(assign_ids_kernel, dim3(grid), dim3(kThreads), 0, c->stream, vals[which], d_flags, d_pos, P,
                     d_off, n, d_ids, d_id_sorted, d_genome_sorted);
  PA_HIP(hipMemcpyAsync(c->h_pinned, d_scalars + 3, sizeof(uint64_t), hipMemcpyDeviceToHost, c->stream));
  PA_HIP(hipStreamSynchronize(c->stream));
  *n_distinct = c->h_pinned[0];
  return PA_OK;
}

int pa_pairs_bitrow(pa_ctx *c, const uint64_t *d_hashes, const uint64_t *d_off, uint32_t n, uint64_t total,
                    uint32_t q0, uint32_t q1, uint32_t s0, uint32_t s1, uint32_t *d_counts) {
  const uint32_t nq = q1 - q0, ns = s1 - s0;
  if (nq == 0 || ns == 0) return PA_OK;
  if (total == 0) {
    PA_HIP(hipMemsetAsync(d_counts, 0, (uint64_t)nq * ns * sizeof(uint32_t), c->stream));
    return PA_OK;
  }
  PA_REQUIRE(total < (1ULL << 32), "pair phase: %llu postings exceed the 32-bit index space",
             (unsigned long long)total);
  const uint64_t P = total;
  uint64_t U = 0;
  PA_TRY(pa_dense_ids_sorted(c, d_hashes, d_off, n, P, &U));
  uint32_t *d_ids = c->ids.as<uint32_t>();
  uint32_t *d_id_sorted = c->post_genome.as<uint32_t>();
  uint32_t *d_genome_sorted = d_id_sorted + P;
  for (uint32_t t0 = s0; t0 < s1; t0 += kMaxTileSubjects) {
    const uint32_t t1 = (s1 - t0 > kMaxTileSubjects) ? t0 + kMaxTileSubjects : s1;
    const uint32_t cols = t1 - t0;
    const int tpr = (int)((cols + 127u) / 128u);
    const uint32_t w32 = (uint32_t)tpr * 4u;
    const uint64_t row_bytes = U * w32 * sizeof(uint32_t);
    {
      ProfScope prof(c, PA_PROF_PAIR_DICT);
      PA_TRY(c->bitrows.reserve(row_bytes));
      PA_HIP(hipMemsetAsync(c->bitrows.p, 0, row_bytes, c->stream));
      hipLaunchKernelGGL(build_rows_kernel, dim3(ceil_div_u64(P, kThreads)), dim3(kThreads), 0, c->stream,
                         d_id_sorted, d_genome_sorted, P, t0, t1, w32, c->bitrows.as<uint32_t>());
    }
    {
      ProfScope prof(c, PA_PROF_PAIR_COUNT);
      const uint32_t *rows = c->bitrows.as<uint32_t>();
      PA_TRY(dispatch_row_sum(c, tpr, nq, d_ids, d_off, q0, rows, cols, d_counts, ns, t0 - s0));
    }
    PA_HIP(hipGetLastError());
  }
  return PA_OK;
}


static int dict_insert(pa_ctx *c, const uint64_t *d_postings, uint64_t n_post, uint32_t *cap_out) {
  const uint64_t cap64 = n_post + n_post / 2 + 1024;
  PA_REQUIRE(cap64 < (1ULL << 32), "pair phase: tile with %llu subject postings is too large for the hash dictionary",
             (unsigned long long)n_post);
  PA_TRY(c->dict_scalars.reserve(64));
  uint32_t *d_counter = c->dict_scalars.as<uint32_t>();
  PA_TRY(c->dict_keys[0].reserve(cap64 * sizeof(DictEntry)));
  PA_HIP(hipMemsetAsync(c->dict_keys[0].p, 0xff, cap64 * sizeof(DictEntry), c->stream));
  PA_HIP(hipMemsetAsync(d_counter, 0, 4, c->stream));
  PA_HIP(hipMemsetAsync(d_counter + 1, 0xff, 4, c->stream));
  if (n_post)
    hipLaunchKernelGGL(table_insert_kernel, dim3(ceil_div_u64(n_post, kThreads * kInsertPerThread)), dim3(kThreads), 0,
                       c->stream, d_postings, (uint64_t)0, n_post, c->dict_keys[0].as<DictEntry>(), (uint32_t)cap64,
                       d_counter, d_counter + 1);
  PA_HIP(hipGetLastError());
  *cap_out = (uint32_t)cap64;
  return PA_OK;
}

int pa_pair_dict_prepare_impl(pa_ctx *c, const uint64_t *d_subject_hashes, uint64_t n_postings) {
  ProfScope prof(c, PA_PROF_PAIR_DICT);
  c->dict_prepared = false;
  uint32_t cap = 0;
  PA_TRY(dict_insert(c, d_subject_hashes, n_postings, &cap));
  unsigned long long *d_fp = c->dict_scalars.as<unsigned long long>() + 1;
  PA_HIP(hipMemsetAsync(d_fp, 0, 16, c->stream));
  if (n_postings)
    hipLaunchKernelGGL(postings_fingerprint_kernel, dim3(std::min<uint32_t>(1024u, ceil_div_u64(n_postings, kThreads))),
                       dim3(kThreads), 0, c->stream, d_subject_hashes, n_postings, d_fp);
  PA_HIP(hipGetLastError());
  c->dict_prepared = true;
  c->dict_prepared_postings = n_postings;
  c->dict_prepared_cap = cap;
  return PA_OK;
}

int pa_pairs_bitrow_hash(pa_ctx *c, const uint64_t *d_hashes, const uint64_t *d_off, const uint64_t *h_off_in,
                         uint32_t n, uint64_t total, uint32_t q0, uint32_t q1, uint32_t s0, uint32_t s1,
                         uint32_t *d_counts) {
  const uint32_t nq = q1 - q0, ns = s1 - s0;
  const bool prepared = c->dict_prepared;
  c->dict_prepared = false;
  if (nq == 0 || ns == 0) return PA_OK;
  if (total == 0) {
    PA_HIP(hipMemsetAsync(d_counts, 0, (uint64_t)nq * ns * sizeof(uint32_t), c->stream));
    return PA_OK;
  }
  PA_REQUIRE(total < (1ULL << 32), "pair phase: %llu postings exceed the 32-bit index space", (unsigned long long)total);
  std::vector<uint64_t> h_off_own;
  const uint64_t *h_off = h_off_in;
  if (!h_off) {
    h_off_own.resize(n + 1);
    PA_HIP(hipMemcpyAsync(h_off_own.data(), d_off, (uint64_t)(n + 1) * 8, hipMemcpyDeviceToHost, c->stream));
    PA_HIP(hipStreamSynchronize(c->stream));
    h_off = h_off_own.data();
  }
  PA_TRY(c->ids.reserve(total * sizeof(uint32_t)));
  PA_TRY(c->dict_scalars.reserve(64));
  uint32_t *d_ids = c->ids.as<uint32_t>();
  uint32_t *d_counter = c->dict_scalars.as<uint32_t>();
  PA_REQUIRE(!prepared || ns <= kMaxTileSubjects, "pair phase: a prepared dictionary serves one tile of at most %u subjects",
             kMaxTileSubjects);
  static const bool symmetry_off = [] { const char *v = PA_TOOL_ENV("PA_PAIRS_SYMMETRIC"); return v && v[0] == '0'; }();
  const bool symmetric = !symmetry_off && q0 == s0 && q1 == s1 && ns > kMaxTileSubjects;
  for (uint32_t t0 = s0; t0 < s1; t0 += kMaxTileSubjects) {
    const uint32_t t1 = (s1 - t0 > kMaxTileSubjects) ? t0 + kMaxTileSubjects : s1;
    const uint32_t cols = t1 - t0;
    const int tpr = (int)((cols + 127u) / 128u);
    const uint32_t w32 = (uint32_t)tpr * 4u;
    const uint32_t tq1 = symmetric ? t1 : q1;
    const uint64_t pt0 = h_off[t0], pt1 = h_off[t1], pq0 = h_off[q0], pq1 = h_off[tq1];
    uint32_t cap = 0;
    {
      ProfScope prof(c, PA_PROF_PAIR_DICT);
      if (prepared) {
        PA_REQUIRE(c->dict_prepared_postings == pt1 - pt0,
                   "pair phase: the prepared dictionary holds %llu postings, the subject tile has %llu",
                   (unsigned long long)c->dict_prepared_postings, (unsigned long long)(pt1 - pt0));
        unsigned long long *d_fp = c->dict_scalars.as<unsigned long long>() + 1;
        PA_HIP(hipMemsetAsync(d_fp + 2, 0, 16, c->stream));
        if (pt1 > pt0)
          hipLaunchKernelGGL(postings_fingerprint_kernel, dim3(std::min<uint32_t>(1024u, ceil_div_u64(pt1 - pt0, kThreads))),
                             dim3(kThreads), 0, c->stream, d_hashes + pt0, pt1 - pt0, d_fp + 2);
        PA_HIP(hipMemcpyAsync(c->h_pinned, d_fp, 32, hipMemcpyDeviceToHost, c->stream));
        PA_HIP(hipStreamSynchronize(c->stream));
        PA_REQUIRE(c->h_pinned[0] == c->h_pinned[2] && c->h_pinned[1] == c->h_pinned[3],
                   "pair phase: the prepared dictionary was built from other postings than the subject tile's "
                   "(same count, %llu, different content)", (unsigned long long)(pt1 - pt0));
        cap = c->dict_prepared_cap;
      } else {
        PA_TRY(dict_insert(c, d_hashes + pt0, pt1 - pt0, &cap));
      }
      constexpr uint64_t kRowBoundBytes = 4ULL << 30;
      uint64_t row_bound = (pt1 - pt0) ? (pt1 - pt0) : 1;
      if (row_bound * w32 * sizeof(uint32_t) > kRowBoundBytes && row_bound * w32 * sizeof(uint32_t) > c->bitrows.bytes) {
        PA_HIP(hipMemcpyAsync(c->h_pinned, d_counter, 8, hipMemcpyDeviceToHost, c->stream));
        PA_HIP(hipStreamSynchronize(c->stream));
        const uint64_t distinct = (uint32_t)c->h_pinned[0];
        row_bound = std::max<uint64_t>(1, std::min<uint64_t>(row_bound, distinct));
      }
      PA_TRY(c->bitrows.reserve(row_bound * w32 * sizeof(uint32_t)));
      hipLaunchKernelGGL(zero_rows_kernel, dim3(ceil_div_u64(row_bound * w32 / 4u, kThreads)), dim3(kThreads), 0,
                         c->stream, c->bitrows.as<uint4>(), d_counter, w32);
      const DictEntry *table = c->dict_keys[0].as<DictEntry>();
      if (pt1 > pt0) {
        uint64_t longest = 0;
        for (uint32_t g = t0; g < t1; ++g) longest = std::max(longest, h_off[g + 1] - h_off[g]);
        hipLaunchKernelGGL(table_lookup_kernel<true>, dim3(ceil_div_u64(longest, kThreads), cols), dim3(kThreads), 0,
                           c->stream, d_hashes, pt0, pt1, table, cap, d_counter + 1, d_ids, d_off, n, t0, w32,
                           c->bitrows.as<uint32_t>());
      }
      const uint64_t a0 = pq0, a1 = pq1 < pt0 ? pq1 : pt0;
      const uint64_t b0 = pq0 > pt1 ? pq0 : pt1, b1 = pq1;
      if (a1 > a0)
        hipLaunchKernelGGL(table_lookup_kernel<false>, dim3(ceil_div_u64(a1 - a0, kThreads)), dim3(kThreads), 0,
                           c->stream, d_hashes, a0, a1, table, cap, d_counter + 1, d_ids, d_off, n, t0, w32,
                           (uint32_t *)nullptr);
      if (b1 > b0)
        hipLaunchKernelGGL(table_lookup_kernel<false>, dim3(ceil_div_u64(b1 - b0, kThreads)), dim3(kThreads), 0,
                           c->stream, d_hashes, b0, b1, table, cap, d_counter + 1, d_ids, d_off, n, t0, w32,
                           (uint32_t *)nullptr);
    }
    {
      ProfScope prof(c, PA_PROF_PAIR_COUNT);
      const uint32_t *rows = c->bitrows.as<uint32_t>();
      PA_TRY(dispatch_row_sum(c, tpr, tq1 - q0, d_ids, d_off, q0, rows, cols, d_counts, ns, t0 - s0));
    }
    PA_HIP(hipGetLastError());
  }
  if (symmetric) {
    ProfScope prof(c, PA_PROF_PAIR_COUNT);
    static_assert(kMaxTileSubjects % 32u == 0, "mirror pieces must not straddle a tile edge");
    const uint32_t g = (ns + 31u) / 32u;
    hipLaunchKernelGGL(mirror_lower_kernel, dim3(g, g), dim3(256), 0, c->stream, d_counts, ns, kMaxTileSubjects);
    PA_HIP(hipGetLastError());
  }
  return PA_OK;
}
```

pyani_plus_amd/csrc/sketch_stream.hip:

```cpp
#include <algorithm>
#include <vector>

#include <cstdlib>

#include "pa_internal.h"

namespace {

constexpr int kThreads = 256;

__global__ __launch_bounds__(kThreads) void mask_from_runs_kernel(const uint64_t *__restrict__ run_start,
                                                                  const uint64_t *__restrict__ run_len, uint32_t n_runs,
                                                                  uint32_t *__restrict__ mask, uint64_t n_words) {
  const uint64_t w = (uint64_t)blockIdx.x * kThreads + threadIdx.x;
  if (w >= n_words) return;
  const uint64_t lo = w * 32u, hi = lo + 32u;
  uint32_t a = 0, b = n_runs;
  while (a < b) {
    const uint32_t mid = (a + b) >> 1;
    if (run_start[mid] + run_len[mid] <= lo) a = mid + 1; else b = mid;
  }
  uint32_t bits = 0;
  for (uint32_t r = a; r < n_runs && run_start[r] < hi; ++r) {
    const uint64_t s = run_start[r] > lo ? run_start[r] : lo;
    const uint64_t e = run_start[r] + run_len[r] < hi ? run_start[r] + run_len[r] : hi;
    if (e > s) {
      const uint32_t n = (uint32_t)(e - s);
      bits |= (n >= 32u ? 0xffffffffu : ((1u << n) - 1u)) << (uint32_t)(s - lo);
    }
  }
  mask[w] = bits;
}

__global__ __launch_bounds__(kThreads) void dirty_kernel(const uint2 *__restrict__ mask, uint64_t n_blocks64,
                                                         uint64_t *__restrict__ dirty) {
  const uint64_t w = ((uint64_t)blockIdx.x * kThreads + threadIdx.x) >> 6;
  const uint64_t t = w * 64u + (threadIdx.x & 63u);
  bool d = false;
  if (t < n_blocks64) {
    const uint2 m = mask[t];
    d = (m.x | m.y) != 0u || t == 0 || mask[t - 1].y != 0u;
  }
  const uint64_t word = __ballot(d);
  if ((threadIdx.x & 63u) == 0 && w * 64u < n_blocks64) dirty[w] = word;
}

}

int pa_build_dirty(pa_ctx *c, const uint32_t *d_mask, uint64_t n_blocks64, uint64_t *d_dirty, hipStream_t stream) {
  if (n_blocks64 == 0) return PA_OK;
  const uint64_t words = (n_blocks64 + 63) / 64;
  hipLaunchKernelGGL(dirty_kernel, dim3(ceil_div_u64(words * 64, kThreads)), dim3(kThreads), 0, stream ? stream : c->stream,
                     reinterpret_cast<const uint2 *>(d_mask), n_blocks64, d_dirty);
  PA_HIP(hipGetLastError());
  return PA_OK;
}

int pa_dirty_or_build(pa_ctx *c, const uint32_t *d_mask, uint64_t n_blocks64, const uint64_t *d_dirty, const uint64_t **out) {
  if (d_dirty) { *out = d_dirty; return PA_OK; }
  PA_TRY(c->dirty.reserve(((n_blocks64 + 63) / 64 + 1) * 8));
  PA_TRY(pa_build_dirty(c, d_mask, n_blocks64, c->dirty.as<uint64_t>()));
  *out = c->dirty.as<uint64_t>();
  return PA_OK;
}

extern "C" {

int pa_arena_dirty(pa_ctx *c, const uint32_t *d_mask, uint64_t arena_bases, uint64_t *d_dirty) {
  PA_REQUIRE(c && (arena_bases == 0 || (d_mask && d_dirty)), "pa_arena_dirty: null argument");
  PA_REQUIRE((arena_bases % PA_ALIGN_BASES) == 0, "pa_arena_dirty: arena_bases %llu is not a multiple of %u",
             (unsigned long long)arena_bases, PA_ALIGN_BASES);
  PA_HIP(hipSetDevice(c->device));
  return pa_build_dirty(c, d_mask, arena_bases / PA_ALIGN_BASES, d_dirty);
}

int pa_mask_from_runs(pa_ctx *c, const uint64_t *h_run_start, const uint64_t *h_run_len, uint32_t n_runs,
                      uint32_t *d_mask, uint64_t arena_bases) {
  PA_REQUIRE(c && (n_runs == 0 || (h_run_start && h_run_len)), "pa_mask_from_runs: null argument");
  PA_REQUIRE((arena_bases % PA_ALIGN_BASES) == 0, "pa_mask_from_runs: arena_bases %llu is not a multiple of %u",
             (unsigned long long)arena_bases, PA_ALIGN_BASES);
  if (arena_bases == 0) return PA_OK;
  PA_REQUIRE(d_mask, "pa_mask_from_runs: null mask");
  PA_HIP(hipSetDevice(c->device));
  for (uint32_t r = 0; r < n_runs; ++r)
    PA_REQUIRE(h_run_len[r] > 0 && h_run_start[r] + h_run_len[r] <= arena_bases &&
                   (r == 0 || h_run_start[r] >= h_run_start[r - 1] + h_run_len[r - 1]),
               "pa_mask_from_runs: run %u is empty, overlaps its predecessor or leaves the arena", r);
  PA_TRY(c->scan_tmp.reserve((uint64_t)n_runs * 16 + 16));
  uint64_t *d_start = c->scan_tmp.as<uint64_t>(), *d_len = d_start + n_runs;
  if (n_runs) {
    PA_HIP(hipMemcpyAsync(d_start, h_run_start, (uint64_t)n_runs * 8, hipMemcpyHostToDevice, c->stream));
    PA_HIP(hipMemcpyAsync(d_len, h_run_len, (uint64_t)n_runs * 8, hipMemcpyHostToDevice, c->stream));
  }
  const uint64_t n_words = arena_bases / 32;
  hipLaunchKernelGGL(mask_from_runs_kernel, dim3(ceil_div_u64(n_words, kThreads)), dim3(kThreads), 0, c->stream, d_start,
                     d_len, n_runs, d_mask, n_words);
  PA_HIP(hipGetLastError());
  PA_HIP(hipStreamSynchronize(c->stream));
  return PA_OK;
}

int pa_sketch_streamed(pa_ctx *c, const uint32_t *h_packed, const uint64_t *h_run_start, const uint64_t *h_run_len,
                       uint32_t n_runs, uint64_t arena_bases, const uint64_t *h_genome_start, uint32_t n_genomes,
                       uint32_t k, uint64_t max_hash, uint32_t *d_packed, uint32_t *d_mask, uint64_t *d_dirty,
                       uint64_t *d_hashes, uint64_t cap_hashes, uint64_t *d_off, uint64_t *h_total) {
  PA_REQUIRE(c && d_off && h_total && h_genome_start, "pa_sketch_streamed: null argument");
  PA_REQUIRE((arena_bases % PA_ALIGN_BASES) == 0, "pa_sketch_streamed: arena_bases %llu is not a multiple of %u",
             (unsigned long long)arena_bases, PA_ALIGN_BASES);
  PA_REQUIRE(arena_bases == 0 || (h_packed && d_packed && d_mask), "pa_sketch_streamed: null arena");
  PA_REQUIRE(k >= 1 && k <= PA_MAX_K, "pa_sketch_streamed: k=%u outside [1,%u]", k, PA_MAX_K);
  PA_REQUIRE(h_genome_start[n_genomes] == arena_bases, "pa_sketch_streamed: genome_start[n] must equal arena_bases");
  PA_HIP(hipSetDevice(c->device));
  *h_total = 0;
  PA_TRY(pa_mask_from_runs(c, h_run_start, h_run_len, n_runs, d_mask, arena_bases));

  const uint64_t n_blocks = arena_bases / PA_ALIGN_BASES;
  if (!d_dirty) {
    PA_TRY(c->dirty.reserve(((n_blocks + 63) / 64 + 1) * 8));
    d_dirty = c->dirty.as<uint64_t>();
  }
  PA_TRY(pa_build_dirty(c, d_mask, n_blocks, d_dirty));
  PA_REQUIRE(n_blocks < (1ULL << 32), "pa_sketch_streamed: arena too large");
  const double frac = (max_hash == UINT64_MAX) ? 1.0 : ((double)max_hash + 1.0) / 18446744073709551616.0;
  std::vector<uint64_t> region_off(n_genomes + 1, 0);
  std::vector<uint32_t> blk(n_genomes + 1);
  uint64_t longest_region = 0;
  for (uint32_t g = 0; g <= n_genomes; ++g) {
    const uint64_t s = h_genome_start[g];
    PA_REQUIRE((s % PA_ALIGN_BASES) == 0 && (g == 0 || s >= h_genome_start[g - 1]) && s <= arena_bases,
               "pa_sketch_streamed: genome_start[%u]=%llu must be an ascending multiple of %u inside the arena", g,
               (unsigned long long)s, PA_ALIGN_BASES);
    blk[g] = (uint32_t)(s / PA_ALIGN_BASES);
    if (g < n_genomes) {
      const uint64_t room = (uint64_t)((double)(h_genome_start[g + 1] - s) * frac * 1.25) + 128;
      longest_region = std::max(longest_region, room);
      region_off[g + 1] = region_off[g] + room;
    }
  }
  const bool overlap = n_genomes > 0 && longest_region <= kLdsSortMax && arena_bases > 0;
  if (!overlap) {
    PA_HIP(hipMemcpyAsync(d_packed, h_packed, arena_bases / 4, hipMemcpyHostToDevice, c->stream));
    return pa_sketch(c, d_packed, d_mask, d_dirty, arena_bases, h_genome_start, n_genomes, k, max_hash, d_hashes, cap_hashes,
                     d_off, h_total);
  }
  if (!c->copy_stream) PA_HIP(hipStreamCreateWithFlags(&c->copy_stream, hipStreamNonBlocking));
  PA_TRY(c->genome_blk.reserve((uint64_t)(n_genomes + 1) * sizeof(uint32_t)));
  PA_TRY(c->region_off.reserve((uint64_t)(n_genomes + 1) * sizeof(uint64_t)));
  PA_TRY(c->region_cursor.reserve((uint64_t)n_genomes * sizeof(uint32_t)));
  PA_TRY(c->cand_keys[0].reserve(region_off[n_genomes] * sizeof(uint64_t)));
  PA_HIP(hipMemcpyAsync(c->genome_blk.p, blk.data(), (uint64_t)(n_genomes + 1) * sizeof(uint32_t), hipMemcpyHostToDevice,
                        c->stream));
  PA_HIP(hipMemcpyAsync(c->region_off.p, region_off.data(), (uint64_t)(n_genomes + 1) * sizeof(uint64_t),
                        hipMemcpyHostToDevice, c->stream));
  uint32_t *d_overflow = c->counters.as<uint32_t>() + 12;
  PA_HIP(hipMemsetAsync(c->region_cursor.p, 0, (uint64_t)n_genomes * sizeof(uint32_t), c->stream));
  PA_HIP(hipMemsetAsync(d_overflow, 0, sizeof(uint32_t), c->stream));
  PA_HIP(hipStreamSynchronize(c->stream));

  uint64_t chunk_blocks = (64ull << 20) / 16;
  if (const char *v = PA_TOOL_ENV("PA_STREAM_CHUNK_BLOCKS"))
    chunk_blocks = std::max<uint64_t>(64, (strtoull(v, nullptr, 10) + 63) / 64 * 64);
  std::vector<hipEvent_t> arrived;
  int status = PA_OK;
  {
    ProfScope prof(c, PA_PROF_KMER_HASH);
    for (uint64_t b0 = 0; b0 < n_blocks && status == PA_OK; b0 += chunk_blocks) {
      const uint64_t b1 = std::min(n_blocks, b0 + chunk_blocks);
      hipEvent_t e;
      if (hipEventCreateWithFlags(&e, hipEventDisableTiming) != hipSuccess) { status = PA_E_HIP; pa_set_error("hipEventCreate failed"); break; }
      arrived.push_back(e);
      if (hipMemcpyAsync(d_packed + b0 * 4, h_packed + b0 * 4, (b1 - b0) * 16, hipMemcpyHostToDevice, c->copy_stream) != hipSuccess ||
          hipEventRecord(e, c->copy_stream) != hipSuccess || hipStreamWaitEvent(c->stream, e, 0) != hipSuccess) {
        status = PA_E_HIP;
        pa_set_error("pa_sketch_streamed: chunk upload failed");
        break;
      }
      status = pa_launch_kmer_hash(c, d_packed, d_mask, d_dirty, b1, c->genome_blk.as<uint32_t>(), n_genomes, k, max_hash,
                                   c->cand_keys[0].as<uint64_t>(), nullptr, 0, nullptr, c->region_off.as<uint64_t>(),
                                   c->region_cursor.as<uint32_t>(), d_overflow, b0, c->stream);
    }
  }
  bool overflow = false;
  if (status == PA_OK) {
    ProfScope prof(c, PA_PROF_SKETCH_SORT);
    status = pa_sketch_from_regions(c, c->cand_keys[0].as<uint64_t>(), c->region_off.as<uint64_t>(),
                                    c->region_cursor.as<uint32_t>(), d_overflow, n_genomes, (uint32_t)longest_region,
                                    max_hash, d_hashes, cap_hashes, d_off, h_total, &overflow);
  } else {
    (void)hipStreamSynchronize(c->copy_stream);
    (void)hipStreamSynchronize(c->stream);
  }
  for (hipEvent_t e : arrived) (void)hipEventDestroy(e);
  if (status != PA_OK) return status;
  if (!overflow) return PA_OK;
  return pa_sketch(c, d_packed, d_mask, d_dirty, arena_bases, h_genome_start, n_genomes, k, max_hash, d_hashes, cap_hashes,
                   d_off, h_total);
}

}
```

Before: 79.25 million.

## Build pair-phase hash dictionary speculatively during k-mer hashing; persistent block walk

The k-mer hash kernel now walks several chunks per block, staging survivors in shared memory and flushing per genome. While it appends sketch candidates it also upserts each hash into the pair-phase dictionary hash table, so the pair phase can adopt that table after a fingerprint check instead of running a separate insert pass. Small metadata uploads go through a cached pinned mirror that skips unchanged re-uploads, and a host stream synchronize is removed. The risks are extra atomics in the hash kernel, a dictionary built from all candidates rather than the final sketch (it is marked speculative, and the pair phase falls back to a normal insert on mismatch), and memset cost for the larger table.

```diff
diff --git a/pyani_plus_amd/csrc/capi.hip b/pyani_plus_amd/csrc/capi.hip
--- a/pyani_plus_amd/csrc/capi.hip
+++ b/pyani_plus_amd/csrc/capi.hip
@@ -35,6 +35,36 @@
   if (!c->prof_on || !e0 || !e1) return;
   (void)hipEventRecord(e1, c->stream);
   c->prof[phase].pending.emplace_back(e0, e1);
+}
+
+int PinnedMirror::upload(void *d_dst, const void *src, uint64_t n_bytes, hipStream_t stream) {
+  if (valid && dev == d_dst && bytes == n_bytes && memcmp(h, src, n_bytes) == 0) return PA_OK;
+  valid = false;
+  if (!copied) PA_HIP(hipEventCreateWithFlags(&copied, hipEventDisableTiming));
+  PA_HIP(hipEventSynchronize(copied));
+  if (n_bytes > cap) {
+    if (h) (void)hipHostFree(h);
+    h = nullptr;
+    cap = 0;
+    const uint64_t want = n_bytes + n_bytes / 4 + 256;
+    if (hipHostMalloc(&h, want, hipHostMallocDefault) != hipSuccess) { h = nullptr; pa_set_error("hipHostMalloc(%llu) failed", (unsigned long long)want); return PA_E_NOMEM; }
+    cap = want;
+  }
+  memcpy(h, src, n_bytes);
+  PA_HIP(hipMemcpyAsync(d_dst, h, n_bytes, hipMemcpyHostToDevice, stream));
+  PA_HIP(hipEventRecord(copied, stream));
+  dev = d_dst;
+  bytes = n_bytes;
+  valid = true;
+  return PA_OK;
+}
+
+void PinnedMirror::release() {
+  if (copied) { (void)hipEventSynchronize(copied); (void)hipEventDestroy(copied); copied = nullptr; }
+  if (h) (void)hipHostFree(h);
+  h = nullptr;
+  cap = bytes = 0;
+  valid = false;
 }
 
 extern "C" {
@@ -88,6 +118,8 @@
                     &c->dict_vals[0], &c->dict_vals[1], &c->ids, &c->post_genome, &c->bitrows, &c->dict_scalars, &c->cls_i, &c->cls_j, &c->cls_score,
                     &c->cls_cov};
   for (DevBuf *b : bufs) b->release();
+  c->genome_blk_host.release();
+  c->region_off_host.release();
   pa_fragani_release(c);
   for (auto &ph : c->prof)
     for (auto &pr : ph.pending) { (void)hipEventDestroy(pr.first); (void)hipEventDestroy(pr.second); }
@@ -184,9 +216,10 @@
     blk[g] = (uint32_t)(s / PA_ALIGN_BASES);
   }
   PA_REQUIRE(n_blocks < (1ULL << 32), "pa_sketch: arena too large");
+  const uint64_t blk_held = c->genome_blk.bytes;
   PA_TRY(c->genome_blk.reserve((uint64_t)(n_genomes + 1) * sizeof(uint32_t)));
-  PA_HIP(hipMemcpyAsync(c->genome_blk.p, blk.data(), (uint64_t)(n_genomes + 1) * sizeof(uint32_t),
-                        hipMemcpyHostToDevice, c->stream));
+  if (c->genome_blk.bytes != blk_held) c->genome_blk_host.valid = false;
+  PA_TRY(c->genome_blk_host.upload(c->genome_blk.p, blk.data(), (uint64_t)(n_genomes + 1) * sizeof(uint32_t), c->stream));
   const double frac = (max_hash == UINT64_MAX) ? 1.0 : ((double)max_hash + 1.0) / 18446744073709551616.0;
   static const bool force_global = [] {
     const char *v = PA_TOOL_ENV("PA_SKETCH_SORT");
@@ -201,25 +234,27 @@
   }
   const bool use_regions = !force_global && n_genomes > 0 && longest_region <= kLdsSortMax;
   if (use_regions) {
+    const uint64_t off_held = c->region_off.bytes;
     PA_TRY(c->region_off.reserve((uint64_t)(n_genomes + 1) * sizeof(uint64_t)));
+    if (c->region_off.bytes != off_held) c->region_off_host.valid = false;
     PA_TRY(c->region_cursor.reserve((uint64_t)n_genomes * sizeof(uint32_t)));
-    PA_HIP(hipMemcpyAsync(c->region_off.p, region_off.data(), (uint64_t)(n_genomes + 1) * sizeof(uint64_t),
-                          hipMemcpyHostToDevice, c->stream));
+    PA_TRY(c->region_off_host.upload(c->region_off.p, region_off.data(), (uint64_t)(n_genomes + 1) * sizeof(uint64_t), c->stream));
   }
   const uint64_t *d_dirty = nullptr;
   PA_TRY(pa_dirty_or_build(c, d_mask, n_blocks, d_dirty_in, &d_dirty));
-  PA_HIP(hipStreamSynchronize(c->stream));
 
   if (use_regions) {
     uint32_t *d_overflow = c->counters.as<uint32_t>() + 12;
     PA_TRY(c->cand_keys[0].reserve(region_off[n_genomes] * sizeof(uint64_t)));
     PA_HIP(hipMemsetAsync(c->region_cursor.p, 0, (uint64_t)n_genomes * sizeof(uint32_t), c->stream));
     PA_HIP(hipMemsetAsync(d_overflow, 0, sizeof(uint32_t), c->stream));
+    PaDictRef dict;
     {
       ProfScope prof(c, PA_PROF_KMER_HASH);
+      PA_TRY(pa_sketch_dict_arm(c, n_genomes, region_off[n_genomes], &dict));
       PA_TRY(pa_launch_kmer_hash(c, d_packed, d_mask, d_dirty, n_blocks, c->genome_blk.as<uint32_t>(), n_genomes, k, max_hash,
                                  c->cand_keys[0].as<uint64_t>(), nullptr, 0, nullptr, c->region_off.as<uint64_t>(),
-                                 c->region_cursor.as<uint32_t>(), d_overflow));
+                                 c->region_cursor.as<uint32_t>(), d_overflow, 0, nullptr, &dict));
     }
     bool overflow = false;
     {
@@ -229,7 +264,10 @@
                                             (uint32_t)longest_region, max_hash, d_hashes, cap_hashes, d_off, h_total, &overflow);
       if (st != PA_OK) return st;
     }
-    if (!overflow) return PA_OK;
+    if (!overflow) {
+      if (dict.table) PA_TRY(pa_sketch_dict_adopt(c, dict, d_hashes, *h_total));
+      return PA_OK;
+    }
     *h_total = 0;
   }
   uint64_t cap = (uint64_t)((double)arena_bases * frac * 1.25) + 65536;
diff --git a/pyani_plus_amd/csrc/dict_dev.h b/pyani_plus_amd/csrc/dict_dev.h
--- /dev/null
+++ b/pyani_plus_amd/csrc/dict_dev.h
@@ -0,0 +1,39 @@
+#pragma once
+
+#include <hip/hip_runtime.h>
+
+#include <cstdint>
+
+namespace pa_dict {
+
+constexpr uint32_t kNone = 0xffffffffu;
+constexpr uint64_t kEmptyKey = ~0ULL;
+
+struct DictEntry {
+  unsigned long long key;
+  uint32_t id;
+  uint32_t pad;
+};
+static_assert(sizeof(DictEntry) == 16, "one probe = one 16-byte entry");
+
+__device__ __forceinline__ uint32_t slot_of(uint64_t h, uint32_t cap) {
+  const uint32_t x = ((uint32_t)h * 0x9E3779B1u) ^ (uint32_t)(h >> 32);
+  return (uint32_t)(((uint64_t)x * cap) >> 32);
+}
+
+__device__ __forceinline__ bool upsert_key(DictEntry *__restrict__ table, uint32_t cap, uint64_t h, uint32_t *won_slot) {
+  uint32_t slot = slot_of(h, cap);
+  for (;;) {
+    unsigned long long k = *reinterpret_cast<volatile const unsigned long long *>(&table[slot].key);
+    if (k == kEmptyKey) k = atomicCAS(&table[slot].key, (unsigned long long)kEmptyKey, (unsigned long long)h);
+    if (k == kEmptyKey) { *won_slot = slot; return true; }
+    if (k == h) return false;
+    if (++slot == cap) slot = 0;
+  }
+}
+
+__device__ __forceinline__ bool upsert_special(uint32_t *__restrict__ special) {
+  return atomicCAS(&special[0], kNone, kNone - 1u) == kNone;
+}
+
+}
diff --git a/pyani_plus_amd/csrc/kmer_hash.hip b/pyani_plus_amd/csrc/kmer_hash.hip
--- a/pyani_plus_amd/csrc/kmer_hash.hip
+++ b/pyani_plus_amd/csrc/kmer_hash.hip
@@ -1,7 +1,9 @@
+#include <algorithm>
 #include <cstdlib>
 #include <type_traits>
 
 #include "pa_internal.h"
+#include "dict_dev.h"
 #include "murmur_dev.h"
 
 namespace {
@@ -22,11 +24,171 @@
   return lo;
 }
 
-__device__ __forceinline__ void region_append(uint64_t *__restrict__ regions, const uint64_t *__restrict__ region_off,
+__device__ __forceinline__ bool region_append(uint64_t *__restrict__ regions, const uint64_t *__restrict__ region_off,
                                               uint32_t *__restrict__ cursor, uint32_t *__restrict__ overflow,
                                               uint32_t g, uint64_t h) {
   const uint64_t slot = atomicAdd(&cursor[g], 1u);
-  if (slot < region_off[g + 1] - region_off[g]) regions[region_off[g] + slot] = h; else *overflow = 1u;
+  const bool fits = slot < region_off[g + 1] - region_off[g];
+  if (fits) regions[region_off[g] + slot] = h; else *overflow = 1u;
+  return fits;
+}
+
+struct Stage {
+  uint64_t hash[kStageCap];
+  uint32_t blk[kStageCap];
+  uint32_t n;
+  unsigned long long base;
+  uint32_t won, id_base;
+};
+
+struct HashOut {
+  const uint32_t *__restrict__ genome_blk;
+  uint32_t n_genomes;
+  uint64_t *__restrict__ cand_hash;
+  uint32_t *__restrict__ cand_genome;
+  uint64_t cap;
+  unsigned long long *__restrict__ count;
+  const uint64_t *__restrict__ region_off;
+  uint32_t *__restrict__ cursor;
+  uint32_t *__restrict__ overflow;
+  pa_dict::DictEntry *__restrict__ dict_table;
+  uint32_t dict_cap;
+  uint32_t *__restrict__ dict_counter;
+};
+
+__device__ __forceinline__ void dict_upsert_one(const HashOut &o, uint64_t h) {
+  uint32_t slot;
+  if (h == pa_dict::kEmptyKey) {
+    if (pa_dict::upsert_special(o.dict_counter + 1)) o.dict_counter[1] = atomicAdd(o.dict_counter, 1u);
+  } else if (pa_dict::upsert_key(o.dict_table, o.dict_cap, h, &slot)) {
+    o.dict_table[slot].id = atomicAdd(o.dict_counter, 1u);
+  }
+}
+
+__device__ __forceinline__ void flush_dict(Stage &s, const HashOut &o, uint32_t n) {
+  constexpr int kPerThread = kStageCap / kThreads;
+  const uint32_t tid = threadIdx.x;
+  uint32_t won_slot[kPerThread];
+  uint32_t won_mask = 0;
+  bool won_special = false;
+#pragma unroll
+  for (int j = 0; j < kPerThread; ++j) {
+    const uint32_t i = tid + (uint32_t)j * kThreads;
+    won_slot[j] = 0;
+    if (i < n) {
+      const uint64_t h = s.hash[i];
+      if (h == pa_dict::kEmptyKey) won_special |= pa_dict::upsert_special(o.dict_counter + 1);
+      else if (pa_dict::upsert_key(o.dict_table, o.dict_cap, h, &won_slot[j])) won_mask |= 1u << j;
+    }
+  }
+  const uint32_t mine = (uint32_t)__builtin_popcount(won_mask) + (won_special ? 1u : 0u);
+  uint32_t local = mine ? atomicAdd(&s.won, mine) : 0u;
+  __syncthreads();
+  if (tid == 0) {
+    s.id_base = s.won ? atomicAdd(o.dict_counter, s.won) : 0u;
+    s.won = 0;
+  }
+  __syncthreads();
+  local += s.id_base;
+#pragma unroll
+  for (int j = 0; j < kPerThread; ++j)
+    if ((won_mask >> j) & 1u) o.dict_table[won_slot[j]].id = local++;
+  if (won_special) o.dict_counter[1] = local;
+}
+
+__device__ __forceinline__ void stage_survivor(Stage &s, const HashOut &o, uint32_t t, uint64_t h) {
+  const uint32_t slot = atomicAdd(&s.n, 1u);
+  if (slot < kStageCap) {
+    s.hash[slot] = h;
+    s.blk[slot] = t;
+  } else if (o.region_off) {
+    const bool fits = region_append(o.cand_hash, o.region_off, o.cursor, o.overflow, find_genome(o.genome_blk, o.n_genomes, t), h);
+    if (fits && o.dict_table) dict_upsert_one(o, h);
+  } else {
+    const unsigned long long g = atomicAdd(o.count, 1ULL);
+    if (g < o.cap) {
+      o.cand_hash[g] = h;
+      o.cand_genome[g] = find_genome(o.genome_blk, o.n_genomes, t);
+    }
+  }
+}
+
+__device__ __forceinline__ void flush_stage(Stage &s, const HashOut &o, uint32_t n, bool one_genome, uint32_t g0) {
+  const uint32_t tid = threadIdx.x;
+  if (o.region_off) {
+    if (one_genome) {
+      if (tid == 0) s.base = atomicAdd(&o.cursor[g0], n);
+      __syncthreads();
+      const uint64_t room = o.region_off[g0 + 1] - o.region_off[g0];
+      uint64_t *__restrict__ dst = o.cand_hash + o.region_off[g0];
+      for (uint32_t i = tid; i < n; i += kThreads) {
+        const uint64_t slot = s.base + i;
+        if (slot < room) dst[slot] = s.hash[i]; else *o.overflow = 1u;
+      }
+      if (o.dict_table) flush_dict(s, o, s.base >= room ? 0u : (uint32_t)min((uint64_t)n, room - s.base));
+    } else {
+      for (uint32_t i = tid; i < n; i += kThreads) {
+        const uint64_t h = s.hash[i];
+        const bool fits = region_append(o.cand_hash, o.region_off, o.cursor, o.overflow, find_genome(o.genome_blk, o.n_genomes, s.blk[i]), h);
+        if (fits && o.dict_table) dict_upsert_one(o, h);
+      }
+    }
+    return;
+  }
+  if (tid == 0) s.base = atomicAdd(o.count, (unsigned long long)n);
+  __syncthreads();
+  const unsigned long long base = s.base;
+  for (uint32_t i = tid; i < n; i += kThreads) {
+    const unsigned long long g = base + i;
+    if (g < o.cap) {
+      o.cand_hash[g] = s.hash[i];
+      o.cand_genome[g] = find_genome(o.genome_blk, o.n_genomes, s.blk[i]);
+    }
+  }
+}
+
+template <typename Body>
+__device__ __forceinline__ void walk_chunks(Stage &s, const HashOut &o, uint32_t blk0, uint32_t n_blocks64,
+                                            uint32_t run_chunks, Body &&body) {
+  const uint32_t tid = threadIdx.x;
+  const uint32_t n_chunks = (uint32_t)(((uint64_t)(n_blocks64 - blk0) + kThreads - 1) / kThreads);
+  const auto last_block = [&](uint32_t chunk) {
+    return (uint32_t)(min((uint64_t)blk0 + ((uint64_t)chunk + 1) * kThreads, (uint64_t)n_blocks64) - 1u);
+  };
+  bool fresh = true, mixed = false;
+  uint32_t g0 = 0, g_end = 0xffffffffu;
+  for (uint64_t run = blockIdx.x; run * run_chunks < n_chunks; run += gridDim.x) {
+    const uint32_t c_end = (uint32_t)min((run + 1) * run_chunks, (uint64_t)n_chunks);
+#pragma unroll 1
+    for (uint32_t ch = (uint32_t)(run * run_chunks); ch < c_end; ++ch) {
+      const uint32_t b0 = blk0 + ch * kThreads;
+      if (o.region_off) {
+        if (fresh) {
+          g0 = find_genome(o.genome_blk, o.n_genomes, b0);
+          g_end = o.genome_blk[g0 + 1];
+          mixed = false;
+        }
+        mixed |= last_block(ch) >= g_end;
+      }
+      fresh = false;
+      const uint32_t t = b0 + tid;
+      if (t < n_blocks64) body(t);
+      const uint64_t next = ch + 1 < c_end ? ch + 1 : (run + gridDim.x) * run_chunks;
+      const bool leaves_genome = next >= n_chunks || last_block((uint32_t)next) >= g_end;
+      __syncthreads();
+      const uint32_t n_raw = __builtin_amdgcn_readfirstlane(s.n);
+      __syncthreads();
+      if (leaves_genome || n_raw > kStageCap / 2) {
+        const uint32_t n = min(n_raw, kStageCap);
+        if (n) {
+          if (tid == 0) s.n = 0;
+          flush_stage(s, o, n, !mixed, g0);
+          __syncthreads();
+        }
+        fresh = true;
+      }
+    }
+  }
 }
 
 template <int K, bool LUT>
@@ -35,12 +197,10 @@
     const uint32_t *__restrict__ genome_blk, uint32_t n_genomes, uint64_t max_hash,
     uint64_t *__restrict__ cand_hash, uint32_t *__restrict__ cand_genome, uint64_t cap,
     unsigned long long *__restrict__ count, const uint64_t *__restrict__ region_off, uint32_t *__restrict__ cursor,
-    uint32_t *__restrict__ overflow, uint32_t blk0) {
+    uint32_t *__restrict__ overflow, uint32_t blk0, uint32_t run_chunks, pa_dict::DictEntry *__restrict__ dict_table,
+    uint32_t dict_cap, uint32_t *__restrict__ dict_counter) {
   static_assert(K >= 1 && K <= 32, "a k-mer is one 64-bit register pair");
-  __shared__ uint64_t s_hash[kStageCap];
-  __shared__ uint32_t s_blk[kStageCap];
-  __shared__ uint32_t s_n;
-  __shared__ unsigned long long s_base;
+  __shared__ Stage s;
   constexpr int kWords = (K + 7) / 8;
   __shared__ uint64_t s_lo[LUT ? kWords : 1][256];
   __shared__ uint32_t s_hi[LUT ? kWords : 1][256];
@@ -49,7 +209,7 @@
   const uint32_t max_hi = (uint32_t)(max_hash >> 32);
   const bool take_all = max_hi == 0xffffffffu;
   const uint32_t screen_hi = max_hi + 1u;
-  if (tid == 0) s_n = 0;
+  if (tid == 0) s.n = s.won = 0;
   if constexpr (LUT) {
 #pragma unroll
     for (int j = 0; j < kWords; ++j) {
@@ -59,9 +219,9 @@
     }
   }
   __syncthreads();
-
-  const uint32_t t = blk0 + blockIdx.x * kThreads + tid;
-  if (t < n_blocks64) {
+  const HashOut o{genome_blk, n_genomes, cand_hash, cand_genome, cap, count, region_off, cursor, overflow, dict_table, dict_cap, dict_counter};
+
+  walk_chunks(s, o, blk0, n_blocks64, run_chunks, [&](const uint32_t t) {
     const uint4 cur = packed[t];
     uint2 pw = make_uint2(0u, 0u);
     if (t > 0) pw = reinterpret_cast<const uint2 *>(packed)[2 * (uint64_t)t - 1];
@@ -139,19 +299,7 @@
             const uint64_t X = U * kF2, Y = V * kF2;
             const uint64_t h = (X ^ (X >> 33)) + (Y ^ (Y >> 33));
             if (h > max_hash || ((bad[wi >> 1] >> (16 * (wi & 1) + i)) & 1u)) continue;
-            const uint32_t slot = atomicAdd(&s_n, 1u);
-            if (slot < kStageCap) {
-              s_hash[slot] = h;
-              s_blk[slot] = t;
-            } else if (region_off) {
-              region_append(cand_hash, region_off, cursor, overflow, find_genome(genome_blk, n_genomes, t), h);
-            } else {
-              const unsigned long long g = atomicAdd(count, 1ULL);
-              if (g < cap) {
-                cand_hash[g] = h;
-                cand_genome[g] = find_genome(genome_blk, n_genomes, t);
-              }
-            }
+            stage_survivor(s, o, t, h);
           }
           }
         }
@@ -160,51 +308,47 @@
       columns(std::integral_constant<int, (kOff0 >> 4)>{}, 0, kSplit);
       if constexpr (kSplit < 16) columns(std::integral_constant<int, (kOff0 >> 4) + 1>{}, kSplit, 16);
     }
-  }
-  __syncthreads();
-  const uint32_t n = min(s_n, kStageCap);
-  if (n == 0) return;
-  if (region_off) {
-    const uint32_t b0 = blk0 + blockIdx.x * kThreads;
-    const uint32_t b1 = min(b0 + (uint32_t)kThreads, n_blocks64) - 1u;
-    const uint32_t g0 = find_genome(genome_blk, n_genomes, b0);
-    if (genome_blk[g0 + 1] > b1) {
-      if (tid == 0) s_base = atomicAdd(&cursor[g0], n);
-      __syncthreads();
-      const uint64_t room = region_off[g0 + 1] - region_off[g0];
-      uint64_t *__restrict__ dst = cand_hash + region_off[g0];
-      for (uint32_t i = tid; i < n; i += kThreads) {
-        const uint64_t slot = s_base + i;
-        if (slot < room) dst[slot] = s_hash[i]; else *overflow = 1u;
-      }
-    } else {
-      for (uint32_t i = tid; i < n; i += kThreads)
-        region_append(cand_hash, region_off, cursor, overflow, find_genome(genome_blk, n_genomes, s_blk[i]), s_hash[i]);
-    }
-    return;
-  }
-  if (tid == 0) s_base = atomicAdd(count, (unsigned long long)n);
-  __syncthreads();
-  const unsigned long long base = s_base;
-  for (uint32_t i = tid; i < n; i += kThreads) {
-    const unsigned long long g = base + i;
-    if (g < cap) {
-      cand_hash[g] = s_hash[i];
-      cand_genome[g] = find_genome(genome_blk, n_genomes, s_blk[i]);
-    }
-  }
+  });
+}
+
+constexpr uint32_t kRunChunks = 4;
+struct WalkGeom { uint32_t grid, run_chunks; };
+template <auto Kern>
+int walk_geometry(pa_ctx *c, uint64_t n_launch_blocks, WalkGeom *out) {
+  static const int per_cu = [] {
+    int n = 0;
+    if (hipOccupancyMaxActiveBlocksPerMultiprocessor(&n, Kern, kThreads, 0) != hipSuccess) n = 0;
+    return n;
+  }();
+  PA_REQUIRE(per_cu > 0, "k-mer hash: the runtime reports no resident workgroup for the kernel");
+  uint32_t run_chunks = kRunChunks;
+  uint64_t grid = (uint64_t)per_cu * (uint64_t)c->prop.multiProcessorCount;
+  bool forced = false;
+  if (const char *v = PA_TOOL_ENV("PA_KMER_RUN")) run_chunks = (uint32_t)std::min<uint64_t>(std::max<uint64_t>(strtoull(v, nullptr, 10), 1), 4096);
+  if (const char *v = PA_TOOL_ENV("PA_KMER_GRID")) {
+    grid = std::min<uint64_t>(std::max<uint64_t>(strtoull(v, nullptr, 10), 1), 1u << 20);
+    forced = true;
+  }
+  const uint64_t n_chunks = (n_launch_blocks + kThreads - 1) / kThreads;
+  const uint64_t n_runs = (n_chunks + run_chunks - 1) / run_chunks;
+  if (!forced) grid = std::min(grid, n_runs);
+  out->grid = (uint32_t)grid;
+  out->run_chunks = run_chunks;
+  return PA_OK;
 }
 
 template <int K, bool LUT>
 int launch_variant(pa_ctx *c, const uint32_t *d_packed, const uint32_t *d_mask, const uint64_t *d_dirty, uint64_t n_blocks64,
            const uint32_t *d_genome_blk, uint32_t n_genomes, uint64_t max_hash, uint64_t *d_cand_hash,
            uint32_t *d_cand_genome, uint64_t cap, uint64_t *d_count, const uint64_t *d_region_off, uint32_t *d_cursor,
-           uint32_t *d_overflow, uint64_t blk0, hipStream_t stream) {
-  const uint32_t grid = ceil_div_u64(n_blocks64 - blk0, kThreads);
-  hipLaunchKernelGGL((kmer_hash_kernel<K, LUT>), dim3(grid), dim3(kThreads), 0, stream ? stream : c->stream,
+           uint32_t *d_overflow, uint64_t blk0, hipStream_t stream, const PaDictRef &dict) {
+  WalkGeom geom;
+  PA_TRY((walk_geometry<&kmer_hash_kernel<K, LUT>>(c, n_blocks64 - blk0, &geom)));
+  hipLaunchKernelGGL((kmer_hash_kernel<K, LUT>), dim3(geom.grid), dim3(kThreads), 0, stream ? stream : c->stream,
                      reinterpret_cast<const uint4 *>(d_packed), reinterpret_cast<const uint2 *>(d_mask), d_dirty,
                      (uint32_t)n_blocks64, d_genome_blk, n_genomes, max_hash, d_cand_hash, d_cand_genome, cap,
-                     reinterpret_cast<unsigned long long *>(d_count), d_region_off, d_cursor, d_overflow, (uint32_t)blk0);
+                     reinterpret_cast<unsigned long long *>(d_count), d_region_off, d_cursor, d_overflow, (uint32_t)blk0,
+                     geom.run_chunks, dict.table, dict.cap, dict.counter);
   PA_HIP(hipGetLastError());
   return PA_OK;
 }
@@ -213,7 +357,7 @@
 int launch(pa_ctx *c, const uint32_t *d_packed, const uint32_t *d_mask, const uint64_t *d_dirty, uint64_t n_blocks64,
            const uint32_t *d_genome_blk, uint32_t n_genomes, uint64_t max_hash, uint64_t *d_cand_hash,
            uint32_t *d_cand_genome, uint64_t cap, uint64_t *d_count, const uint64_t *d_region_off, uint32_t *d_cursor,
-           uint32_t *d_overflow, uint64_t blk0, hipStream_t stream) {
+           uint32_t *d_overflow, uint64_t blk0, hipStream_t stream, const PaDictRef &dict) {
   static const bool arithmetic = [] {
     const char *v = PA_TOOL_ENV("PA_KMER_VARIANT");
     return v && v[0] == '0';
@@ -221,9 +365,9 @@
   if constexpr (K == 31)
     if (arithmetic)
       return launch_variant<K, false>(c, d_packed, d_mask, d_dirty, n_blocks64, d_genome_blk, n_genomes, max_hash, d_cand_hash,
-                                    d_cand_genome, cap, d_count, d_region_off, d_cursor, d_overflow, blk0, stream);
+                                    d_cand_genome, cap, d_count, d_region_off, d_cursor, d_overflow, blk0, stream, dict);
   return launch_variant<K, true>(c, d_packed, d_mask, d_dirty, n_blocks64, d_genome_blk, n_genomes, max_hash, d_cand_hash,
-                                 d_cand_genome, cap, d_count, d_region_off, d_cursor, d_overflow, blk0, stream);
+                                 d_cand_genome, cap, d_count, d_region_off, d_cursor, d_overflow, blk0, stream, dict);
 }
 
 template <int K>
@@ -232,12 +376,10 @@
     const uint32_t *__restrict__ genome_blk, uint32_t n_genomes, uint64_t max_hash,
     uint64_t *__restrict__ cand_hash, uint32_t *__restrict__ cand_genome, uint64_t cap,
     unsigned long long *__restrict__ count, const uint64_t *__restrict__ region_off, uint32_t *__restrict__ cursor,
-    uint32_t *__restrict__ overflow, uint32_t blk0) {
+    uint32_t *__restrict__ overflow, uint32_t blk0, uint32_t run_chunks, pa_dict::DictEntry *__restrict__ dict_table,
+    uint32_t dict_cap, uint32_t *__restrict__ dict_counter) {
   static_assert(K >= 33 && K <= 64, "k-mers of 65 to 128 bits");
-  __shared__ uint64_t s_hash[kStageCap];
-  __shared__ uint32_t s_blk[kStageCap];
-  __shared__ uint32_t s_n;
-  __shared__ unsigned long long s_base;
+  __shared__ Stage s;
   constexpr int kWords = (K + 7) / 8;
   __shared__ uint64_t s_lo[kWords][256];
   __shared__ uint32_t s_hi[kWords][256];
@@ -245,7 +387,7 @@
   const uint32_t max_hi = (uint32_t)(max_hash >> 32);
   const bool take_all = max_hi == 0xffffffffu;
   const uint32_t screen_hi = max_hi + 1u;
-  if (tid == 0) s_n = 0;
+  if (tid == 0) s.n = s.won = 0;
 #pragma unroll
   for (int j = 0; j < kWords; ++j) {
     const uint64_t cj = (j & 1) ? kC2 : kC1;
@@ -253,9 +395,9 @@
     s_hi[j][tid] = (uint32_t)((uint64_t)ascii_group(tid, K - 8 * j - 4) * cj);
   }
   __syncthreads();
-
-  const uint32_t t = blk0 + blockIdx.x * kThreads + tid;
-  if (t < n_blocks64) {
+  const HashOut o{genome_blk, n_genomes, cand_hash, cand_genome, cap, count, region_off, cursor, overflow, dict_table, dict_cap, dict_counter};
+
+  walk_chunks(s, o, blk0, n_blocks64, run_chunks, [&](const uint32_t t) {
     const uint4 cur = packed[t];
     const uint4 prev = t > 0 ? packed[t - 1] : make_uint4(0u, 0u, 0u, 0u);
     uint32_t d2 = 0u, d3 = 0u;
@@ -336,19 +478,7 @@
               const uint64_t X = U * kF2, Y = V * kF2;
               const uint64_t h = (X ^ (X >> 33)) + (Y ^ (Y >> 33));
               if (h > max_hash || ((bad[wi >> 1] >> (16 * (wi & 1) + i)) & 1u)) continue;
-              const uint32_t slot = atomicAdd(&s_n, 1u);
-              if (slot < kStageCap) {
-                s_hash[slot] = h;
-                s_blk[slot] = t;
-              } else if (region_off) {
-                region_append(cand_hash, region_off, cursor, overflow, find_genome(genome_blk, n_genomes, t), h);
-              } else {
-                const unsigned long long g = atomicAdd(count, 1ULL);
-                if (g < cap) {
-                  cand_hash[g] = h;
-                  cand_genome[g] = find_genome(genome_blk, n_genomes, t);
-                }
-              }
+              stage_survivor(s, o, t, h);
             }
           }
         }
@@ -357,39 +487,7 @@
       columns(std::integral_constant<int, (kOff0 >> 4)>{}, 0, kSplit);
       if constexpr (kSplit < 16) columns(std::integral_constant<int, (kOff0 >> 4) + 1>{}, kSplit, 16);
     }
-  }
-  __syncthreads();
-  const uint32_t n = min(s_n, kStageCap);
-  if (n == 0) return;
-  if (region_off) {
-    const uint32_t b0 = blk0 + blockIdx.x * kThreads;
-    const uint32_t b1 = min(b0 + (uint32_t)kThreads, n_blocks64) - 1u;
-    const uint32_t g0 = find_genome(genome_blk, n_genomes, b0);
-    if (genome_blk[g0 + 1] > b1) {
-      if (tid == 0) s_base = atomicAdd(&cursor[g0], n);
-      __syncthreads();
-      const uint64_t room = region_off[g0 + 1] - region_off[g0];
-      uint64_t *__restrict__ dst = cand_hash + region_off[g0];
-      for (uint32_t i = tid; i < n; i += kThreads) {
-        const uint64_t slot = s_base + i;
-        if (slot < room) dst[slot] = s_hash[i]; else *overflow = 1u;
-      }
-    } else {
-      for (uint32_t i = tid; i < n; i += kThreads)
-        region_append(cand_hash, region_off, cursor, overflow, find_genome(genome_blk, n_genomes, s_blk[i]), s_hash[i]);
-    }
-    return;
-  }
-  if (tid == 0) s_base = atomicAdd(count, (unsigned long long)n);
-  __syncthreads();
-  const unsigned long long base = s_base;
-  for (uint32_t i = tid; i < n; i += kThreads) {
-    const unsigned long long g = base + i;
-    if (g < cap) {
-      cand_hash[g] = s_hash[i];
-      cand_genome[g] = find_genome(genome_blk, n_genomes, s_blk[i]);
-    }
-  }
+  });
 }
 
 __device__ __forceinline__ uint32_t rev_groups32(uint32_t x) {
@@ -404,10 +502,10 @@
   for (uint32_t i = 0; i < 4; ++i) {
     if (i >= nblocks) break;
     h1 ^= rotl64(P[2 * i], 31) * kC2;
-    h1 = rotl64(h1, 27) + h2;
+    h1 = add64(rotl64(h1, 27), h2);
     h1 = times5_plus(h1, 0x52dce729ULL);
     h2 ^= rotl64(P[2 * i + 1], 33) * kC1;
-    h2 = rotl64(h2, 31) + h1;
+    h2 = add64(rotl64(h2, 31), h1);
     h2 = times5_plus(h2, 0x38495ab5ULL);
   }
   uint64_t t1 = 0, t2 = 0;
@@ -515,20 +613,23 @@
                         const uint32_t *d_genome_blk, uint32_t n_genomes, uint32_t k, uint64_t max_hash,
                         uint64_t *d_cand_hash, uint32_t *d_cand_genome, uint64_t cap, uint64_t *d_count,
                         const uint64_t *d_region_off, uint32_t *d_cursor, uint32_t *d_overflow, uint64_t blk0,
-                        hipStream_t stream) {
+                        hipStream_t stream, const PaDictRef *dict_in) {
+  const PaDictRef dict = dict_in ? *dict_in : PaDictRef{};
   PA_REQUIRE(n_blocks64 < (1ULL << 32), "arena too large: %llu blocks of 64 bases", (unsigned long long)n_blocks64);
   if (n_blocks64 <= blk0) return PA_OK;
   const char *long_form = PA_TOOL_ENV("PA_KMER_LONG");
   const bool long_plain = long_form && long_form[0] == 'p';
   if (k > 32 && k <= 64 && !long_plain) {
     PA_REQUIRE((blk0 & 63u) == 0, "k-mer hash launch must start at a multiple of 64 blocks, not %llu", (unsigned long long)blk0);
-    const uint32_t grid = ceil_div_u64(n_blocks64 - blk0, kThreads);
+    WalkGeom geom;
 #define PA_WIDE_CASE(KK)                                                                                                   \
   case KK:                                                                                                                 \
-    hipLaunchKernelGGL((kmer_hash_wide_kernel<KK>), dim3(grid), dim3(kThreads), 0, stream ? stream : c->stream,            \
+    PA_TRY((walk_geometry<&kmer_hash_wide_kernel<KK>>(c, n_blocks64 - blk0, &geom)));                                      \
+    hipLaunchKernelGGL((kmer_hash_wide_kernel<KK>), dim3(geom.grid), dim3(kThreads), 0, stream ? stream : c->stream,       \
                        reinterpret_cast<const uint4 *>(d_packed), reinterpret_cast<const uint2 *>(d_mask), d_dirty,        \
                        (uint32_t)n_blocks64, d_genome_blk, n_genomes, max_hash, d_cand_hash, d_cand_genome, cap,           \
-                       reinterpret_cast<unsigned long long *>(d_count), d_region_off, d_cursor, d_overflow, (uint32_t)blk0); \
+                       reinterpret_cast<unsigned long long *>(d_count), d_region_off, d_cursor, d_overflow, (uint32_t)blk0, \
+                       geom.run_chunks, dict.table, dict.cap, dict.counter);                                               \
     break;
     switch (k) {
       PA_WIDE_CASE(33) PA_WIDE_CASE(34) PA_WIDE_CASE(35) PA_WIDE_CASE(36) PA_WIDE_CASE(37) PA_WIDE_CASE(38) PA_WIDE_CASE(39)
@@ -556,7 +657,7 @@
     return PA_OK;
   }
 #define PA_K_CASE(KK) \
-  case KK: return launch<KK>(c, d_packed, d_mask, d_dirty, n_blocks64, d_genome_blk, n_genomes, max_hash, d_cand_hash, d_cand_genome, cap, d_count, d_region_off, d_cursor, d_overflow, blk0, stream);
+  case KK: return launch<KK>(c, d_packed, d_mask, d_dirty, n_blocks64, d_genome_blk, n_genomes, max_hash, d_cand_hash, d_cand_genome, cap, d_count, d_region_off, d_cursor, d_overflow, blk0, stream, dict);
   PA_REQUIRE((blk0 & 63u) == 0, "k-mer hash launch must start at a multiple of 64 blocks, not %llu", (unsigned long long)blk0);
   switch (k) {
     PA_K_CASE(1) PA_K_CASE(2) PA_K_CASE(3) PA_K_CASE(4) PA_K_CASE(5) PA_K_CASE(6) PA_K_CASE(7) PA_K_CASE(8)
diff --git a/pyani_plus_amd/csrc/murmur_dev.h b/pyani_plus_amd/csrc/murmur_dev.h
--- a/pyani_plus_amd/csrc/murmur_dev.h
+++ b/pyani_plus_amd/csrc/murmur_dev.h
@@ -42,6 +42,12 @@
   return t + c;
 }
 
+__device__ __forceinline__ uint64_t add64(uint64_t a, uint64_t b) {
+  uint64_t d;
+  asm("v_lshl_add_u64 %0, %1, 0, %2" : "=v"(d) : "v"(a), "v"(b));
+  return d;
+}
+
 constexpr uint64_t kF1 = 0xff51afd7ed558ccdULL, kF2 = 0xc4ceb9fe1a85ec53ULL;
 
 template <int K, int N>
@@ -57,12 +63,12 @@
     if (i == 0) {
       h1 = times5_plus(rotl64(h1, 27), 5ULL * 42ULL + 0x52dce729ULL);
     } else {
-      h1 = rotl64(h1, 27) + h2;
+      h1 = add64(rotl64(h1, 27), h2);
       h1 = times5_plus(h1, 0x52dce729ULL);
     }
     const uint64_t k2 = rotl64(P[2 * i + 1], 33) * kC1;
     h2 ^= k2;
-    h2 = rotl64(h2, 31) + h1;
+    h2 = add64(rotl64(h2, 31), h1);
     h2 = times5_plus(h2, 0x38495ab5ULL);
   }
   if constexpr (tail > 8) h2 ^= rotl64(P[2 * nblocks + 1], 33) * kC1;
diff --git a/pyani_plus_amd/csrc/pa_internal.h b/pyani_plus_amd/csrc/pa_internal.h
--- a/pyani_plus_amd/csrc/pa_internal.h
+++ b/pyani_plus_amd/csrc/pa_internal.h
@@ -90,6 +90,23 @@
   T *as() const { return reinterpret_cast<T *>(p); }
 };
 
+struct PinnedMirror {
+  void *h = nullptr;
+  uint64_t cap = 0, bytes = 0;
+  const void *dev = nullptr;
+  bool valid = false;
+  hipEvent_t copied = nullptr;
+  int upload(void *d_dst, const void *src, uint64_t n_bytes, hipStream_t stream);
+  void release();
+};
+
+namespace pa_dict { struct DictEntry; }
+struct PaDictRef {
+  pa_dict::DictEntry *table = nullptr;
+  uint32_t cap = 0;
+  uint32_t *counter = nullptr;
+};
+
 struct ProfPhase {
   double total_ms = 0.0;
   uint64_t launches = 0;
@@ -108,9 +125,11 @@
   DevBuf flags, scan_tmp;
   DevBuf region_off, region_cursor;
   DevBuf dirty;
+  PinnedMirror genome_blk_host, region_off_host;
   DevBuf dict_keys[2], dict_vals[2];
   DevBuf ids, post_genome, bitrows;
   bool dict_prepared = false;
+  bool dict_speculative = false;
   uint64_t dict_prepared_postings = 0;
   uint32_t dict_prepared_cap = 0;
   DevBuf dict_scalars;
@@ -144,7 +163,8 @@
                         const uint32_t *d_genome_blk, uint32_t n_genomes, uint32_t k, uint64_t max_hash,
                         uint64_t *d_cand_hash, uint32_t *d_cand_genome, uint64_t cap, uint64_t *d_count,
                         const uint64_t *d_region_off = nullptr, uint32_t *d_cursor = nullptr,
-                        uint32_t *d_overflow = nullptr, uint64_t blk0 = 0, hipStream_t stream = nullptr);
+                        uint32_t *d_overflow = nullptr, uint64_t blk0 = 0, hipStream_t stream = nullptr,
+                        const PaDictRef *dict = nullptr);
 
 int pa_build_dirty(pa_ctx *c, const uint32_t *d_mask, uint64_t n_blocks64, uint64_t *d_dirty, hipStream_t stream = nullptr);
 int pa_dirty_or_build(pa_ctx *c, const uint32_t *d_mask, uint64_t n_blocks64, const uint64_t *d_dirty, const uint64_t **out);
@@ -166,6 +186,8 @@
                          uint32_t n, uint64_t total, uint32_t q0, uint32_t q1, uint32_t s0, uint32_t s1,
                          uint32_t *d_counts);
 int pa_pair_dict_prepare_impl(pa_ctx *c, const uint64_t *d_subject_hashes, uint64_t n_postings);
+int pa_sketch_dict_arm(pa_ctx *c, uint32_t n_genomes, uint64_t bound, PaDictRef *out);
+int pa_sketch_dict_adopt(pa_ctx *c, const PaDictRef &dict, const uint64_t *d_hashes, uint64_t n_postings);
 int pa_pairs_merge(pa_ctx *c, const uint64_t *d_hashes, const uint64_t *d_off, uint32_t n, uint32_t q0,
                    uint32_t q1, uint32_t s0, uint32_t s1, uint32_t *d_counts);
 
diff --git a/pyani_plus_amd/csrc/pairs_bitrow.hip b/pyani_plus_amd/csrc/pairs_bitrow.hip
--- a/pyani_plus_amd/csrc/pairs_bitrow.hip
+++ b/pyani_plus_amd/csrc/pairs_bitrow.hip
@@ -3,14 +3,15 @@
 #include <vector>
 
 #include "pa_internal.h"
+#include "dict_dev.h"
 
 namespace {
+
+using namespace pa_dict;
 
 constexpr int kThreads = 256;
 constexpr int kPlanes = 10;
 constexpr uint32_t kMaxTileSubjects = 2048;
-constexpr uint32_t kNone = 0xffffffffu;
-constexpr uint64_t kEmptyKey = ~0ULL;
 
 __global__ __launch_bounds__(kThreads) void iota_kernel(uint32_t *__restrict__ vals, uint64_t n) {
   const uint64_t i = (uint64_t)blockIdx.x * kThreads + threadIdx.x;
@@ -176,18 +177,6 @@
   if (i < n16) rows[i] = make_uint4(0u, 0u, 0u, 0u);
 }
 
-struct DictEntry {
-  unsigned long long key;
-  uint32_t id;
-  uint32_t pad;
-};
-static_assert(sizeof(DictEntry) == 16, "one probe = one 16-byte entry");
-
-__device__ __forceinline__ uint32_t slot_of(uint64_t h, uint32_t cap) {
-  const uint32_t x = ((uint32_t)h * 0x9E3779B1u) ^ (uint32_t)(h >> 32);
-  return (uint32_t)(((uint64_t)x * cap) >> 32);
-}
-
 constexpr int kInsertPerThread = 4;
 __global__ __launch_bounds__(kThreads) void table_insert_kernel(const uint64_t *__restrict__ hashes, uint64_t p0,
                                                                 uint64_t p1, DictEntry *__restrict__ table,
@@ -206,17 +195,11 @@
     if (p >= p1) break;
     const uint64_t h = hashes[p];
     if (h == kEmptyKey) {
-      won_special = atomicCAS(&special[0], kNone, kNone - 1u) == kNone;
+      won_special |= upsert_special(special);
       continue;
     }
-    uint32_t slot = slot_of(h, cap);
-    for (;;) {
-      unsigned long long k = *reinterpret_cast<volatile const unsigned long long *>(&table[slot].key);
-      if (k == kEmptyKey) k = atomicCAS(&table[slot].key, (unsigned long long)kEmptyKey, (unsigned long long)h);
-      if (k == kEmptyKey) { won_slot[won++] = slot; break; }
-      if (k == h) break;
-      if (++slot == cap) slot = 0;
-    }
+    uint32_t slot;
+    if (upsert_key(table, cap, h, &slot)) won_slot[won++] = slot;
   }
   const uint32_t mine = (uint32_t)won + (won_special ? 1u : 0u);
   uint32_t local = mine ? atomicAdd(&s_won, mine) : 0u;
@@ -431,8 +414,42 @@
                        dim3(kThreads), 0, c->stream, d_subject_hashes, n_postings, d_fp);
   PA_HIP(hipGetLastError());
   c->dict_prepared = true;
+  c->dict_speculative = false;
   c->dict_prepared_postings = n_postings;
   c->dict_prepared_cap = cap;
+  return PA_OK;
+}
+
+int pa_sketch_dict_arm(pa_ctx *c, uint32_t n_genomes, uint64_t bound, PaDictRef *out) {
+  *out = PaDictRef{};
+  const char *sw = PA_TOOL_ENV("PA_SKETCH_DICT");
+  if ((sw && sw[0] == '0') || n_genomes == 0 || n_genomes > kMaxTileSubjects) return PA_OK;
+  const uint64_t cap64 = bound + bound / 2 + 1024;
+  if (cap64 >= (1ULL << 32)) return PA_OK;
+  c->dict_prepared = false;
+  PA_TRY(c->dict_scalars.reserve(64));
+  uint32_t *d_counter = c->dict_scalars.as<uint32_t>();
+  PA_TRY(c->dict_keys[0].reserve(cap64 * sizeof(DictEntry)));
+  PA_HIP(hipMemsetAsync(c->dict_keys[0].p, 0xff, cap64 * sizeof(DictEntry), c->stream));
+  PA_HIP(hipMemsetAsync(d_counter, 0, 4, c->stream));
+  PA_HIP(hipMemsetAsync(d_counter + 1, 0xff, 4, c->stream));
+  out->table = c->dict_keys[0].as<DictEntry>();
+  out->cap = (uint32_t)cap64;
+  out->counter = d_counter;
+  return PA_OK;
+}
+
+int pa_sketch_dict_adopt(pa_ctx *c, const PaDictRef &dict, const uint64_t *d_hashes, uint64_t n_postings) {
+  unsigned long long *d_fp = c->dict_scalars.as<unsigned long long>() + 1;
+  PA_HIP(hipMemsetAsync(d_fp, 0, 16, c->stream));
+  if (n_postings)
+    hipLaunchKernelGGL(postings_fingerprint_kernel, dim3(std::min<uint32_t>(1024u, ceil_div_u64(n_postings, kThreads))),
+                       dim3(kThreads), 0, c->stream, d_hashes, n_postings, d_fp);
+  PA_HIP(hipGetLastError());
+  c->dict_prepared = true;
+  c->dict_speculative = true;
+  c->dict_prepared_postings = n_postings;
+  c->dict_prepared_cap = dict.cap;
   return PA_OK;
 }
 
@@ -440,7 +457,8 @@
                          uint32_t n, uint64_t total, uint32_t q0, uint32_t q1, uint32_t s0, uint32_t s1,
                          uint32_t *d_counts) {
   const uint32_t nq = q1 - q0, ns = s1 - s0;
-  const bool prepared = c->dict_prepared;
+  bool prepared = c->dict_prepared;
+  const bool speculative = prepared && c->dict_speculative;
   c->dict_prepared = false;
   if (nq == 0 || ns == 0) return PA_OK;
   if (total == 0) {
@@ -460,6 +478,7 @@
   PA_TRY(c->dict_scalars.reserve(64));
   uint32_t *d_ids = c->ids.as<uint32_t>();
   uint32_t *d_counter = c->dict_scalars.as<uint32_t>();
+  if (speculative && (ns > kMaxTileSubjects || c->dict_prepared_postings != h_off[s1] - h_off[s0])) prepared = false;
   PA_REQUIRE(!prepared || ns <= kMaxTileSubjects, "pair phase: a prepared dictionary serves one tile of at most %u subjects",
              kMaxTileSubjects);
   static const bool symmetry_off = [] { const char *v = PA_TOOL_ENV("PA_PAIRS_SYMMETRIC"); return v && v[0] == '0'; }();
@@ -485,13 +504,13 @@
                              dim3(kThreads), 0, c->stream, d_hashes + pt0, pt1 - pt0, d_fp + 2);
         PA_HIP(hipMemcpyAsync(c->h_pinned, d_fp, 32, hipMemcpyDeviceToHost, c->stream));
         PA_HIP(hipStreamSynchronize(c->stream));
-        PA_REQUIRE(c->h_pinned[0] == c->h_pinned[2] && c->h_pinned[1] == c->h_pinned[3],
+        const bool same = c->h_pinned[0] == c->h_pinned[2] && c->h_pinned[1] == c->h_pinned[3];
+        PA_REQUIRE(same || speculative,
                    "pair phase: the prepared dictionary was built from other postings than the subject tile's "
                    "(same count, %llu, different content)", (unsigned long long)(pt1 - pt0));
-        cap = c->dict_prepared_cap;
-      } else {
-        PA_TRY(dict_insert(c, d_hashes + pt0, pt1 - pt0, &cap));
+        if (same) cap = c->dict_prepared_cap; else prepared = false;
       }
+      if (!prepared) PA_TRY(dict_insert(c, d_hashes + pt0, pt1 - pt0, &cap));
       constexpr uint64_t kRowBoundBytes = 4ULL << 30;
       uint64_t row_bound = (pt1 - pt0) ? (pt1 - pt0) : 1;
       if (row_bound * w32 * sizeof(uint32_t) > kRowBoundBytes && row_bound * w32 * sizeof(uint32_t) > c->bitrows.bytes) {
diff --git a/pyani_plus_amd/csrc/sketch_stream.hip b/pyani_plus_amd/csrc/sketch_stream.hip
--- a/pyani_plus_amd/csrc/sketch_stream.hip
+++ b/pyani_plus_amd/csrc/sketch_stream.hip
@@ -148,6 +148,7 @@
   PA_TRY(c->region_off.reserve((uint64_t)(n_genomes + 1) * sizeof(uint64_t)));
   PA_TRY(c->region_cursor.reserve((uint64_t)n_genomes * sizeof(uint32_t)));
   PA_TRY(c->cand_keys[0].reserve(region_off[n_genomes] * sizeof(uint64_t)));
+  c->genome_blk_host.valid = c->region_off_host.valid = false;
   PA_HIP(hipMemcpyAsync(c->genome_blk.p, blk.data(), (uint64_t)(n_genomes + 1) * sizeof(uint32_t), hipMemcpyHostToDevice,
                         c->stream));
   PA_HIP(hipMemcpyAsync(c->region_off.p, region_off.data(), (uint64_t)(n_genomes + 1) * sizeof(uint64_t),
```

Result: slower. 70.97 million (-10.4%).
